# twosigma/Cook

Hardware: AMD Instinct MI355X
Metric: match-cycles/sec at 1M pending x 50k offers (higher is better)
Workload: dtype f64

## Files before the change

### cook_amd/csrc/classfit_asm.hpp

```cpp
#pragma once
#if CF_SLOTS_N == 12
#define CF_O_CTRL "13728"
#define CF_O_CTRL4 "13732"
#define CF_O_ARR "15280"
#define CF_O_CLS32 "9504"
#define CF_SLOT_SHIFT "9"
#define CF_SLOT_N "12"
#elif CF_SLOTS_N == 24
#define CF_O_CTRL "16800"
#define CF_O_CTRL4 "16804"
#define CF_O_ARR "18352"
#define CF_O_CLS32 "12576"
#define CF_SLOT_SHIFT "10"
#define CF_SLOT_N "24"
#else
#error "CF_SLOTS_N: 12 or 24"
#endif
#ifndef CF_ASM_WAIT_READS
#define CF_ASM_WAIT_READS "30"
#endif
#define CF_ASM_MAX_STEP(ctrl) "v_max_f32_dpp v113, v113, v113 " ctrl "\n\ts_nop 1\n\t"
#define CF_ASM_DECIDER_STEP                                                                                                             \
  "v_readlane_b32 s60, v80, s44\n\t"                                                                                                    \
  "v_readlane_b32 s61, v81, s44\n\t"                                                                                                    \
  "v_readlane_b32 s62, v82, s44\n\t"                                                                                                    \
  "s_mov_b32 s41, 1\n\t"                                                                                                                \
  "s_and_b32 s63, s62, 0xffff00ff\n\t"                                                                                                   \
  "s_cmp_lg_u32 s63, 0\n\t"                                                                                                             \
  "s_cbranch_scc1 9f\n\t"                                                                                                               \
                                                                                           \
  "v_mov_b32_e32 v88, s47\n\t"                                                                                                          \
  "v_mov_b32_e32 v89, s51\n\t"                                                                                                          \
  "v_add_u32_e32 v100, s46, v83\n\t"                                                                                                    \
  "s_mov_b64 exec, 1\n\t"                                                                                                               \
  "ds_write_b32 v89, v88 offset:" CF_O_CTRL4 "\n\t"                                                                                              \
  "s_mov_b64 exec, -1\n\t"                                                                                                              \
  "s_mov_b32 s82, " CF_ASM_WAIT_READS "\n\t"              \
  "1:\n\t"                                                                                                                              \
  "ds_read_b32 v92, v100\n\t"                                                                                                           \
  "ds_read_b64 v[94:95], v100 offset:8\n\t"                                                                                             \
  "ds_read_b128 v[96:99], v100 offset:16\n\t"                                                                                           \
  "ds_read_b32 v93, v100\n\t"                                                                                                           \
  "v_lshlrev_b32_e32 v114, 3, v65\n\t"  \
  "v_add_u32_e32 v114, s56, v114\n\t"                                                                                                   \
  "ds_read_b64 v[114:115], v114\n\t"                                                                                                    \
                                        \
  "v_subrev_u32_e32 v101, s60, v71\n\t"                                                                                                 \
  "v_subrev_u32_e32 v102, s61, v72\n\t"                                                                                                 \
  "v_cvt_f64_u32_e32 v[104:105], v101\n\t"                                                                                              \
  "v_cvt_f64_u32_e32 v[106:107], v102\n\t"                                                                                              \
  "v_mul_f64 v[104:105], v[104:105], v[66:67]\n\t"                                                                                      \
  "v_mul_f64 v[106:107], v[106:107], v[68:69]\n\t"                                                                                      \
  "v_add_f64 v[104:105], v[104:105], v[106:107]\n\t"                                                                                    \
  "v_add_f64 v[104:105], -v[104:105], 1.0\n\t"                                                                                          \
  "v_cmp_le_u32_e64 s[64:65], s60, v71\n\t"                                                                                             \
  "v_cmp_le_u32_e64 s[66:67], s61, v72\n\t"                                                                                             \
  "v_cmp_ne_u32_e64 s[68:69], 0, v64\n\t"                                                                                               \
  "s_and_b64 s[64:65], s[64:65], s[66:67]\n\t"                                                                                          \
  "s_and_b64 s[64:65], s[64:65], s[68:69]\n\t"                                                                                          \
  "s_waitcnt lgkmcnt(0)\n\t"                                                                                                            \
        \
  "s_bfe_u32 s63, s62, 0x4000c\n\t"                                                                                                     \
  "s_cmp_eq_u32 s63, 0\n\t"                                                                                                             \
  "s_cbranch_scc1 3f\n\t"                                                                                                               \
  "v_readlane_b32 s66, v85, s44\n\t"                                                                                                    \
  "v_readlane_b32 s67, v86, s44\n\t"                                                                                                    \
  "s_cmp_lt_u32 s63, 1\n\t"                                                                                                           \
  "s_cbranch_scc1 3f\n\t"                                                                                                               \
  "s_bfe_u32 s72, s66, 0x100000\n\t"                                                                      \
  "s_lshr_b32 s73, s72, 8\n\t"                                                                                                          \
  "s_lshl_b32 s73, s73, 3\n\t"                                                                                                          \
  "s_and_b32 s72, s72, 0xff\n\t"                                                                                                        \
  "v_lshrrev_b64 v[108:109], s73, v[114:115]\n\t"                                                                                       \
  "v_and_b32_e32 v108, 0xff, v108\n\t"                                                                                                  \
  "v_cmp_eq_u32_e64 s[74:75], s72, v108\n\t"                                                                                            \
  "s_and_b64 s[64:65], s[64:65], s[74:75]\n\t"                                                                                          \
  "s_cmp_lt_u32 s63, 2\n\t"                                                                                                           \
  "s_cbranch_scc1 3f\n\t"                                                                                                               \
  "s_bfe_u32 s72, s66, 0x100010\n\t"                                                                      \
  "s_lshr_b32 s73, s72, 8\n\t"                                                                                                          \
  "s_lshl_b32 s73, s73, 3\n\t"                                                                                                          \
  "s_and_b32 s72, s72, 0xff\n\t"                                                                                                        \
  "v_lshrrev_b64 v[108:109], s73, v[114:115]\n\t"                                                                                       \
  "v_and_b32_e32 v108, 0xff, v108\n\t"                                                                                                  \
  "v_cmp_eq_u32_e64 s[74:75], s72, v108\n\t"                                                                                            \
  "s_and_b64 s[64:65], s[64:65], s[74:75]\n\t"                                                                                          \
  "s_cmp_lt_u32 s63, 3\n\t"                                                                                                           \
  "s_cbranch_scc1 3f\n\t"                                                                                                               \
  "s_bfe_u32 s72, s67, 0x100000\n\t"                                                                      \
  "s_lshr_b32 s73, s72, 8\n\t"                                                                                                          \
  "s_lshl_b32 s73, s73, 3\n\t"                                                                                                          \
  "s_and_b32 s72, s72, 0xff\n\t"                                                                                                        \
  "v_lshrrev_b64 v[108:109], s73, v[114:115]\n\t"                                                                                       \
  "v_and_b32_e32 v108, 0xff, v108\n\t"                                                                                                  \
  "v_cmp_eq_u32_e64 s[74:75], s72, v108\n\t"                                                                                            \
  "s_and_b64 s[64:65], s[64:65], s[74:75]\n\t"                                                                                          \
  "s_cmp_lt_u32 s63, 4\n\t"                                                                                                           \
  "s_cbranch_scc1 3f\n\t"                                                                                                               \
  "s_bfe_u32 s72, s67, 0x100010\n\t"                                                                      \
  "s_lshr_b32 s73, s72, 8\n\t"                                                                                                          \
  "s_lshl_b32 s73, s73, 3\n\t"                                                                                                          \
  "s_and_b32 s72, s72, 0xff\n\t"                                                                                                        \
  "v_lshrrev_b64 v[108:109], s73, v[114:115]\n\t"                                                                                       \
  "v_and_b32_e32 v108, 0xff, v108\n\t"                                                                                                  \
  "v_cmp_eq_u32_e64 s[74:75], s72, v108\n\t"                                                                                            \
  "s_and_b64 s[64:65], s[64:65], s[74:75]\n\t"                                                                                          \
  "3:\n\t"                                                                                                                              \
   \
  "v_and_b32_e32 v108, 0xffffff00, v92\n\t"                                                                                             \
  "v_cmp_eq_u32_e64 s[70:71], s45, v108\n\t"                                                                                            \
  "v_cmp_eq_u32_e64 s[72:73], v92, v93\n\t"                                                                                             \
  "v_sub_u32_e32 v108, v73, v92\n\t"                                                                                                    \
  "v_and_b32_e32 v108, 0xff, v108\n\t"                                                                                                  \
  "v_cmp_gt_u32_e64 s[74:75], 3, v108\n\t"                                                                                              \
  "v_and_b32_e32 v109, 0xffff, v94\n\t"                                                                                                 \
  "v_cmp_ne_u32_e64 s[76:77], v109, v74\n\t"                                                                                            \
  "v_cmp_ne_u32_e64 s[78:79], v109, v75\n\t"                                                                                            \
  "v_cmp_gt_i32_e64 s[80:81], 0, v95\n\t"                                                                                               \
  "s_and_b64 s[74:75], s[74:75], s[76:77]\n\t"                                                                                          \
  "s_and_b64 s[74:75], s[74:75], s[78:79]\n\t"                                                                                          \
  "s_or_b64 s[74:75], s[74:75], s[80:81]\n\t"                                                                                           \
  "s_and_b64 s[72:73], s[70:71], s[72:73]\n\t"                                          \
  "s_and_b64 s[70:71], s[72:73], s[74:75]\n\t"                                                                                            \
  "s_andn2_b64 s[76:77], s[52:53], s[70:71]\n\t"                                                                     \
  "s_cmp_eq_u64 s[76:77], 0\n\t"                                                                                                          \
  "s_cbranch_scc1 2f\n\t"                                                                                                                 \
   \
   \
  "s_and_b64 s[78:79], s[76:77], s[72:73]\n\t"                                                                                            \
  "s_cmp_eq_u64 s[78:79], 0\n\t"                                                                                                          \
  "s_cbranch_scc1 4f\n\t"                                                                                                                 \
  "v_and_b32_e32 v109, 0x3fff, v95\n\t"                                                                                                   \
  "s_and_b64 s[72:73], s[64:65], s[54:55]\n\t"                                                   \
  "10:\n\t"                                                                                                                               \
  "s_ff1_i32_b64 s83, s[78:79]\n\t"                                                                                                       \
  "v_readlane_b32 s63, v109, s83\n\t"                                                                                                     \
  "s_bitset0_b64 s[78:79], s83\n\t"                                                                                                       \
  "v_cmp_eq_u32_e64 vcc, s63, v65\n\t"                                                                                                    \
  "s_and_b64 vcc, vcc, s[72:73]\n\t"                                                                                                      \
  "s_cmp_eq_u64 vcc, 0\n\t"                                                                                                               \
  "s_cbranch_scc1 11f\n\t"                                                                                                                \
  "s_bitset1_b64 s[80:81], s83\n\t"                                                                                                       \
  "s_bitset0_b64 s[76:77], s83\n\t"                                                                                                       \
  "11:\n\t"                                                                                                                               \
  "s_cmp_lg_u64 s[78:79], 0\n\t"                                                                                                          \
  "s_cbranch_scc1 10b\n\t"                                                                                                                \
  "s_cmp_eq_u64 s[76:77], 0\n\t"                                                                                                          \
  "s_cbranch_scc1 2f\n\t"                                                                                                                 \
  "4:\n\t"                                                                                                                                \
  "s_sub_u32 s82, s82, 1\n\t"      \
  "s_cmp_eq_u32 s82, 0\n\t"                                                                                                             \
  "s_cbranch_scc1 9f\n\t"                                                                                                               \
  "s_sleep 1\n\t"                                                                                                                       \
  "s_branch 1b\n\t"                                                                                                                     \
  "2:\n\t"                                                                                                                              \
  "s_andn2_b64 s[74:75], s[52:53], s[80:81]\n\t"                                                                        \
  "s_or_b64 s[64:65], s[64:65], s[74:75]\n\t"                                                          \
  "v_cndmask_b32_e64 v110, v98, v104, s[54:55]\n\t"                                                                                     \
  "v_cndmask_b32_e64 v111, v99, v105, s[54:55]\n\t"                                                                                     \
  "v_cndmask_b32_e64 v110, 0, v110, s[64:65]\n\t"                                                                                       \
  "v_cndmask_b32_e64 v111, 0, v111, s[64:65]\n\t"                                                                                       \
  "v_cvt_f32_f64_e32 v112, v[110:111]\n\t"                                                                                              \
  "s_nop 0\n\t"                                                                                                                         \
  "v_mov_b32_e32 v113, v112\n\t"                                                                                                        \
  "s_nop 1\n\t"                                                                                                                         \
  CF_ASM_MAX_STEP("quad_perm:[1,0,3,2] row_mask:0xf bank_mask:0xf")                                                                     \
  CF_ASM_MAX_STEP("quad_perm:[2,3,0,1] row_mask:0xf bank_mask:0xf")                                                                     \
  CF_ASM_MAX_STEP("row_half_mirror row_mask:0xf bank_mask:0xf")                                                                         \
  CF_ASM_MAX_STEP("row_mirror row_mask:0xf bank_mask:0xf")                                                                              \
  CF_ASM_MAX_STEP("row_bcast:15 row_mask:0xa bank_mask:0xf")                                                                            \
  CF_ASM_MAX_STEP("row_bcast:31 row_mask:0xc bank_mask:0xf")                                                                            \
  "v_readlane_b32 s63, v113, 63\n\t"                                                                                                    \
  "s_mov_b32 s41, 0\n\t"                                                                                                                \
  "s_cmp_eq_u32 s63, 0\n\t"                                                                                                             \
  "s_cbranch_scc1 9f\n\t"                                                                                          \
  "s_mov_b32 s41, 1\n\t"                                                                                                                \
  "v_cmp_eq_f32_e64 s[78:79], s63, v112\n\t"                                                                                            \
  "v_add_f32_e32 v108, 0x35000000, v112\n\t"                                                                               \
  "v_cmp_le_f32_e64 s[76:77], s63, v108\n\t"                                                                                            \
  "v_and_b32_e32 v109, 0x40000000, v95\n\t"                                                                                             \
  "v_cmp_ne_u32_e64 s[70:71], 0, v109\n\t"                                                                                              \
  "s_and_b64 s[76:77], s[76:77], s[64:65]\n\t"                                      \
  "s_bcnt1_i32_b64 s62, s[76:77]\n\t"                                                                                                   \
  "s_cmp_gt_u32 s62, 1\n\t"                                                                                                             \
  "s_cbranch_scc1 9f\n\t"                                                                                                               \
  "s_and_b64 s[70:71], s[70:71], s[76:77]\n\t"                                                                                          \
  "s_and_b64 s[70:71], s[70:71], s[74:75]\n\t"                       \
  "s_cmp_lg_u64 s[70:71], 0\n\t"                                                                                                        \
  "s_cbranch_scc1 9f\n\t"                                                                                                               \
  "s_ff1_i32_b64 s82, s[78:79]\n\t"                                                                                                     \
  "s_cmp_lt_u32 s82, 58\n\t"                                                                                                            \
  "s_cbranch_scc0 5f\n\t"                                                                                                               \
                                                                                                         \
  "v_readlane_b32 s64, v71, s82\n\t"                                                                                                    \
  "v_readlane_b32 s65, v72, s82\n\t"                                                                                                    \
  "v_readlane_b32 s66, v65, s82\n\t"                                                                                                    \
  "s_sub_u32 s67, s64, s60\n\t"                                                                                                         \
  "s_sub_u32 s70, s65, s61\n\t"                                                                                                         \
  "v_cmp_eq_u32_e64 vcc, s82, v84\n\t"                                                                                                  \
  "v_mov_b32_e32 v88, s67\n\t"                                                                                                          \
  "v_mov_b32_e32 v89, s70\n\t"                                                                                                          \
  "s_cmp_lt_u32 s67, s49\n\t"                                                                                                           \
  "s_cselect_b32 s71, 1, 0\n\t"                                                                                                         \
  "s_cmp_lt_u32 s70, s50\n\t"                                                                                                           \
  "s_cselect_b32 s62, 1, 0\n\t"                                                                                                         \
  "s_or_b32 s71, s71, s62\n\t"                                                                                                          \
  "v_cndmask_b32_e32 v71, v71, v88, vcc\n\t"                                                                                            \
  "v_cndmask_b32_e32 v72, v72, v89, vcc\n\t"                                                                                            \
  "s_cmp_lg_u32 s71, 0\n\t"                                                                                                             \
  "s_cselect_b64 s[62:63], vcc, 0\n\t"                             \
  "s_mov_b32 s72, s44\n\t"                                                                                                              \
  "s_mov_b32 s73, 0\n\t"                                                                                                                \
  "v_cndmask_b32_e64 v64, v64, 0, s[62:63]\n\t"                                                                                         \
  "s_branch 7f\n\t"                                                                                                                     \
        \
  "5:\n\t"                                                                                                                              \
  "v_readlane_b32 s64, v96, s82\n\t"                                                                                                    \
  "v_readlane_b32 s65, v97, s82\n\t"                                                                                                    \
  "v_readlane_b32 s76, v95, s82\n\t"                                                                                                    \
  "v_readlane_b32 s77, v94, s82\n\t"                                                                                                    \
  "v_readlane_b32 s78, v73, s82\n\t"                                                                                                    \
  "s_sub_u32 s67, s64, s60\n\t"                                                                                                         \
  "s_sub_u32 s70, s65, s61\n\t"                                                                                                         \
  "s_and_b32 s66, s76, 0x3fff\n\t"                                                                                                      \
  "s_bfe_u32 s79, s76, 0x80010\n\t"                                                                                                     \
  "s_and_b32 s73, s77, 0xffff\n\t"                                                                                                      \
  "s_lshr_b32 s81, s77, 16\n\t"                                                                                                         \
  "s_sub_u32 s80, s82, 57\n\t"                                                                                                          \
  "s_cmp_lt_u32 s67, s49\n\t"                                                                                                           \
  "s_cselect_b32 s71, 1, 0\n\t"                                                                                                         \
  "s_cmp_lt_u32 s70, s50\n\t"                                                                                                           \
  "s_cselect_b32 s62, 1, 0\n\t"                                                                                                         \
  "s_or_b32 s71, s71, s62\n\t"                                                                                                          \
  "s_bcnt1_i32_b64 s62, s[68:69]\n\t"                                                                                                   \
  "s_cmp_lg_u32 s71, 0\n\t"                                                                                                             \
  "s_cbranch_scc1 6f\n\t"                                                                                                               \
  "s_cmp_ge_u32 s62, " CF_ASM_EPOCH_LIVE "\n\t"                                                                                          \
  "s_cbranch_scc1 9f\n\t"                                  \
  "6:\n\t"                                                                                                                              \
  "s_lshl_b32 s62, s73, 3\n\t"                                                                                                          \
  "s_add_u32 s62, s62, s51\n\t"                                                                                                         \
  "s_lshl_b32 s63, s80, 2\n\t"                                                                                                          \
  "s_add_u32 s63, s63, s51\n\t"                                                                                                         \
  "s_add_u32 s78, s78, 1\n\t"                                                                                                           \
  "v_mov_b32_e32 v88, 0\n\t"                                                                                                            \
  "v_mov_b32_e32 v89, 0\n\t"                                                                                                            \
  "v_mov_b32_e32 v90, s62\n\t"                                                                                                          \
  "v_mov_b32_e32 v91, s63\n\t"                                                                                                          \
  "v_mov_b32_e32 v100, s78\n\t"                                                                                                         \
  "s_mov_b64 exec, 1\n\t"                                                                                                               \
  "ds_write_b64 v90, v[88:89] offset:" CF_O_ARR "\n\t"                                                                                         \
  "ds_write_b32 v91, v100 offset:" CF_O_CTRL4 "\n\t"                                                                                             \
  "s_mov_b64 exec, -1\n\t"                                                                                                              \
  "v_cmp_eq_u32_e64 vcc, s82, v84\n\t"                                                                                                  \
  "v_mov_b32_e32 v101, s73\n\t"                                                                                                         \
  "s_nop 0\n\t"                                                                                                                         \
  "v_cndmask_b32_e32 v75, v75, v74, vcc\n\t"                                                                                            \
  "v_cndmask_b32_e32 v74, v74, v101, vcc\n\t"                                                                                           \
  "v_cndmask_b32_e32 v73, v73, v100, vcc\n\t"                                                                                           \
  "s_lshl_b32 s62, s80, 8\n\t"                                                                                                          \
  "s_lshl_b32 s63, s81, 12\n\t"                                                                                                         \
  "s_or_b32 s72, s44, s62\n\t"                                                                                                          \
  "s_or_b32 s72, s72, s63\n\t"                                                                                                          \
  "s_cmp_lg_u32 s71, 0\n\t"                                                                                                             \
  "s_cbranch_scc1 7f\n\t"                                                                              \
  "s_mul_i32 s62, s79, 56\n\t"                                                                                                          \
  "s_add_u32 s62, s62, s51\n\t"                                                                                                         \
  "v_mov_b32_e32 v90, s62\n\t"                                                                                                          \
  "ds_read_b128 v[116:119], v90 offset:" CF_O_CLS32 "\n\t"                                                                                        \
  "s_andn2_b64 s[62:63], s[54:55], s[68:69]\n\t"                                                                                        \
  "s_ff1_i32_b64 s83, s[62:63]\n\t"                                                                                                     \
  "v_cmp_eq_u32_e64 vcc, s83, v84\n\t"                                                                                                  \
  "v_mov_b32_e32 v88, s66\n\t"                                                                                                          \
  "v_mov_b32_e32 v89, s79\n\t"                                                                                                          \
  "v_mov_b32_e32 v91, s67\n\t"                                                                                                          \
  "v_mov_b32_e32 v101, s70\n\t"                                                                                                         \
  "v_cndmask_b32_e64 v64, v64, 1, vcc\n\t"                                                                                              \
  "v_cndmask_b32_e32 v65, v65, v88, vcc\n\t"                                                                                            \
  "v_cndmask_b32_e32 v70, v70, v89, vcc\n\t"                                                                                            \
  "v_cndmask_b32_e32 v71, v71, v91, vcc\n\t"                                                                                            \
  "v_cndmask_b32_e32 v72, v72, v101, vcc\n\t"                                                                                           \
  "s_waitcnt lgkmcnt(0)\n\t"                                                                                                            \
  "v_cndmask_b32_e32 v66, v66, v116, vcc\n\t"                                                                                           \
  "v_cndmask_b32_e32 v67, v67, v117, vcc\n\t"                                                                                           \
  "v_cndmask_b32_e32 v68, v68, v118, vcc\n\t"                                                                                           \
  "v_cndmask_b32_e32 v69, v69, v119, vcc\n\t"                                                                                           \
   \
  "7:\n\t"                                                                                                                              \
  "v_cmp_eq_u32_e64 vcc, s44, v84\n\t"                                                                                                  \
  "v_mov_b32_e32 v88, s66\n\t"                                                                                                          \
  "v_cmp_lt_u32_e64 s[62:63], s67, v80\n\t"                                                                                             \
  "v_cmp_lt_u32_e64 s[76:77], s70, v81\n\t"                                                                                             \
  "v_cndmask_b32_e32 v76, v76, v88, vcc\n\t"                                                                                            \
  "s_or_b64 s[62:63], s[62:63], s[76:77]\n\t"                                                                                           \
  "s_lshl_b64 s[76:77], -2, s44\n\t"                                                                                                    \
  "s_and_b64 s[62:63], s[62:63], s[76:77]\n\t"                                                                                          \
  "s_or_b64 s[38:39], s[38:39], s[62:63]\n\t"                                                                                           \
  "s_min_u32 s37, s37, s67\n\t"                                                                                                         \
  "s_min_u32 s40, s40, s70\n\t"                                                                                                         \
  "s_add_u32 s36, s36, 1\n\t"                                                                                                           \
  "v_mov_b32_e32 v88, s72\n\t"                                                                                                          \
  "v_mov_b32_e32 v89, s73\n\t"                                                                                                          \
  "v_mov_b32_e32 v90, s64\n\t"                                                                                                          \
  "v_mov_b32_e32 v91, s65\n\t"                                                                                                          \
  "v_mov_b32_e32 v100, s48\n\t"                                                                                                         \
  "s_mov_b64 exec, 1\n\t"                                                                                                               \
  "ds_write_b128 v100, v[88:91]\n\t"                                                                                                    \
  "s_mov_b64 exec, -1\n\t"                                                                                                              \
  "s_mov_b32 s41, 2\n\t"                                                                                                                \
  "9:\n\t"

#define CF_ASM_CLASS_STEP                                                                                                               \
  "v_mov_b32_e32 v80, s44\n\t"                                                                                                          \
  "s_lshl_b32 s60, s45, 2\n\t"                                                                                                          \
  "s_add_u32 s60, s60, s44\n\t"                                                                                                         \
  "v_mov_b32_e32 v81, s60\n\t"                                                                                                          \
  "ds_read_b64 v[82:83], v80 offset:" CF_O_CTRL "\n\t"                                                                     \
  "ds_read_b32 v84, v81 offset:" CF_O_CTRL4 "\n\t"                                                                   \
  "s_mov_b32 s41, 3\n\t"                                                                                                                \
  "s_waitcnt lgkmcnt(0)\n\t"                                                                                                            \
  "v_readfirstlane_b32 s61, v82\n\t"                                                                                                    \
  "v_readfirstlane_b32 s42, v83\n\t"                                                                                                    \
  "v_readfirstlane_b32 s43, v84\n\t"                                                                                                    \
  "s_cmp_lg_u32 s61, 0\n\t"                                                                                                             \
  "s_cbranch_scc1 9f\n\t"                                                                                                               \
  "s_cmp_lg_u32 s43, s40\n\t"                                                                                                           \
  "s_cbranch_scc1 9f\n\t"                                                                                                               \
  "s_mov_b32 s41, 2\n\t"                                                                                                                \
                                                                                                 \
  "1:\n\t"                                                                                                                              \
  "s_cmp_eq_u64 s[36:37], 0\n\t"                                                                                                        \
  "s_cbranch_scc1 9f\n\t"                                                                                                               \
  "s_cmp_eq_u32 s39, s56\n\t"                                                                                                           \
  "s_cbranch_scc1 2f\n\t"                                                                                                               \
  "s_add_u32 s62, s36, -1\n\t"                                                                                                          \
  "s_addc_u32 s63, s37, -1\n\t"                                                                                                         \
  "s_and_b64 s[36:37], s[36:37], s[62:63]\n\t"                                                                                          \
  "s_add_u32 s38, s38, 1\n\t"                                                                                                           \
  "s_add_u32 s39, s39, 1\n\t"                                                                                                           \
  "s_cmp_eq_u32 s39, s57\n\t"                                                                                                           \
  "s_cselect_b32 s39, 0, s39\n\t"                                                                                                       \
  "s_branch 1b\n\t"                                                                                                                     \
  "2:\n\t"                                                                                                                                \
  "s_lshr_b32 s60, s42, 8\n\t"                                                                                                            \
  "s_cmp_lt_u32 s38, s60\n\t"                                          \
  "s_cbranch_scc0 12f\n\t"                                                                                                                \
  "s_mov_b32 s41, 3\n\t"                                                                                                                  \
  "s_branch 9f\n\t"                                                                                                                       \
  "12:\n\t"                                                                                                                               \
  "s_add_u32 s60, s60, s59\n\t"                                                                                                         \
  "s_cmp_ge_u32 s38, s60\n\t"                                                                                                           \
  "s_cbranch_scc1 9f\n\t"                                                                             \
  "s_ff1_i32_b64 s64, s[36:37]\n\t"                                                                                                     \
  "v_readlane_b32 s65, v72, s64\n\t"                                                                                                    \
  "v_readlane_b32 s66, v73, s64\n\t"                                                                                                    \
  "v_readlane_b32 s67, v74, s64\n\t"                                                                                                    \
  "s_mov_b32 s41, 1\n\t"                                                                                                                \
  "s_lshr_b32 s60, s67, 12\n\t"                                                                                                         \
  "s_cmp_lg_u32 s60, 0\n\t"                                                                                                             \
  "s_cbranch_scc1 9f\n\t"                                                                                \
  "s_and_b32 s60, s67, 0xff\n\t"                                                                                                        \
  "s_cmp_lg_u32 s60, s58\n\t"                                                                                                           \
  "s_cbranch_scc1 8f\n\t"                                                                                \
                                           \
  "s_bfe_u32 s60, s67, 0x30008\n\t"                                                                                                     \
  "s_bitcmp1_b32 s60, 0\n\t"                                                                                                            \
  "s_cselect_b64 vcc, -1, 0\n\t"                                                                                                        \
  "v_cndmask_b32_e32 v80, v64, v65, vcc\n\t"                                                                                            \
  "v_cndmask_b32_e32 v81, v66, v67, vcc\n\t"                                                                                            \
  "v_cndmask_b32_e32 v82, v68, v69, vcc\n\t"                                                                                            \
  "v_cndmask_b32_e32 v83, v70, v71, vcc\n\t"                                                                                            \
  "s_bitcmp1_b32 s60, 1\n\t"                                                                                                            \
  "s_cselect_b64 vcc, -1, 0\n\t"                                                                                                        \
  "v_cndmask_b32_e32 v80, v80, v81, vcc\n\t"                                                                                            \
  "v_cndmask_b32_e32 v82, v82, v83, vcc\n\t"                                                                                            \
  "s_bitcmp1_b32 s60, 2\n\t"                                                                                                            \
  "s_cselect_b64 vcc, -1, 0\n\t"                                                                                                        \
  "v_cndmask_b32_e32 v80, v80, v82, vcc\n\t"                                                                                            \
                                                                 \
  "s_mul_i32 s68, s38, 43\n\t"                                                                                                          \
  "s_lshr_b32 s68, s68, " CF_SLOT_SHIFT "\n\t"                                                                                                          \
  "s_mul_i32 s68, s68, " CF_SLOT_N "\n\t"                                                                                                          \
  "s_sub_u32 s68, s38, s68\n\t"                                                                                                         \
  "s_lshl_b32 s68, s68, 8\n\t"                                                                                                          \
  "s_lshl_b32 s69, s45, 5\n\t"                                                                                                          \
  "s_add_u32 s68, s68, s69\n\t"                                                                                                         \
  "s_add_u32 s68, s68, s44\n\t"                                                                                                         \
  "s_add_u32 s69, s46, s64\n\t"                                                                                                         \
  "s_lshl_b32 s69, s69, 12\n\t"                                                                                                         \
  "s_or_b32 s69, s69, s47\n\t"                                                                                                          \
  "s_and_b32 s70, s40, 0xff\n\t"                                                                                                        \
  "s_or_b32 s69, s69, s70\n\t"                                                                                                          \
  "v_mov_b32_e32 v94, s68\n\t"                                                                                                          \
  "v_mov_b32_e32 v95, s69\n\t"                                                                                                          \
  "v_mov_b32_e32 v96, -1\n\t"                                                                                                           \
  "v_cmp_lt_u32_e64 s[70:71], s66, v80\n\t"                                                 \
  "s_cmp_eq_u64 s[70:71], 0\n\t"                                                                                                        \
  "s_cbranch_scc1 6f\n\t"                                                                                                               \
  "s_ff1_i32_b64 s72, s[70:71]\n\t"                                                                                                     \
  "s_lshl_b32 s73, s72, 6\n\t"                                                                                                          \
  "s_add_u32 s74, s73, s48\n\t"                                                                        \
  "s_sub_u32 s75, s49, s73\n\t"                                                                              \
  "v_add_u32_e32 v97, s74, v75\n\t"                                                                                                     \
  "v_lshlrev_b32_e32 v98, 3, v97\n\t"                                                                                                   \
  "v_add_u32_e32 v98, s44, v98\n\t"                                                                                                     \
  "v_lshlrev_b32_e32 v99, 1, v97\n\t"                                                                                                   \
  "v_add_u32_e32 v99, s50, v99\n\t"                                                                                                     \
  "ds_read_b64 v[84:85], v98 offset:" CF_O_ARR "\n\t"                                                                                          \
  "ds_read_u16 v90, v99\n\t"                                                                                                            \
  "s_waitcnt lgkmcnt(0)\n\t"                                                                                                            \
  "v_cmp_le_u32_e64 s[76:77], s65, v84\n\t"                                                                                             \
  "v_cmp_le_u32_e64 s[78:79], s66, v85\n\t"                                                                                             \
  "v_cmp_gt_u32_e64 s[80:81], s75, v75\n\t"                                                                                             \
  "v_and_b32_e32 v91, 0x8000, v90\n\t"                                                                                                  \
  "v_cmp_eq_u32_e64 s[82:83], 0, v91\n\t"                                                                                               \
  "s_and_b64 s[76:77], s[76:77], s[78:79]\n\t"                                                                                          \
  "s_and_b64 s[76:77], s[76:77], s[80:81]\n\t"                                                                                          \
  "s_and_b64 s[76:77], s[76:77], s[82:83]\n\t"                                                                                          \
  "s_cmp_eq_u64 s[76:77], 0\n\t"                                                                                                        \
  "s_cbranch_scc1 9f\n\t"               \
                                                    \
  "v_subrev_u32_e32 v91, s65, v84\n\t"                                                                                                  \
  "v_subrev_u32_e32 v92, s66, v85\n\t"                                                                                                  \
  "v_cvt_f64_u32_e32 v[86:87], v91\n\t"                                                                                                 \
  "v_cvt_f64_u32_e32 v[88:89], v92\n\t"                                                                                                 \
  "v_mul_f64 v[86:87], v[86:87], s[52:53]\n\t"                                                                                          \
  "v_mul_f64 v[88:89], v[88:89], s[54:55]\n\t"                                                                                          \
  "v_add_f64 v[86:87], v[86:87], v[88:89]\n\t"                                                                                          \
  "v_add_f64 v[86:87], -v[86:87], 1.0\n\t"                                                                                              \
  "v_mov_b32_e32 v91, s72\n\t"                                                                                                          \
  "v_lshl_or_b32 v92, v91, 16, v97\n\t"                                                                \
  "v_and_b32_e32 v93, 0x3fff, v90\n\t"                                                                                                  \
  "v_or_b32_e32 v93, s51, v93\n\t"                                                                                                      \
  "v_lshlrev_b32_e32 v91, 16, v90\n\t"                                                                                                  \
  "v_and_b32_e32 v91, 0x40000000, v91\n\t"                              \
  "v_or_b32_e32 v93, v93, v91\n\t"                                                                                                      \
  "s_ff1_i32_b64 s78, s[76:77]\n\t"                                                                                                     \
  "s_lshl_b64 s[78:79], 1, s78\n\t"                                                                                                     \
  "s_mov_b64 exec, s[78:79]\n\t"                                                                                                        \
  "ds_write_b32 v94, v96\n\t"                                                                                                           \
  "ds_write_b128 v94, v[84:87] offset:16\n\t"                                                                                           \
  "ds_write_b64 v94, v[92:93] offset:8\n\t"                                                                                             \
  "ds_write_b32 v94, v95\n\t"                                                                                                           \
  "s_mov_b64 exec, -1\n\t"                                                                                                              \
  "s_branch 8f\n\t"                                                                                                                     \
                                                                                                    \
  "6:\n\t"                                                                                                                              \
  "v_mov_b32_e32 v92, 0\n\t"                                                                                                            \
  "v_mov_b32_e32 v93, 0x80000000\n\t"                                                                                                   \
  "s_mov_b64 exec, 1\n\t"                                                                                                               \
  "ds_write_b32 v94, v96\n\t"                                                                                                           \
  "ds_write_b64 v94, v[92:93] offset:8\n\t"                                                                                             \
  "ds_write_b32 v94, v95\n\t"                                                                                                           \
  "s_mov_b64 exec, -1\n\t"                                                                                                              \
                                                                                                              \
  "8:\n\t"                                                                                                                              \
  "s_add_u32 s62, s36, -1\n\t"                                                                                                          \
  "s_addc_u32 s63, s37, -1\n\t"                                                                                                         \
  "s_and_b64 s[36:37], s[36:37], s[62:63]\n\t"                                                                                          \
  "s_add_u32 s38, s38, 1\n\t"                                                                                                           \
  "s_add_u32 s39, s39, 1\n\t"                                                                                                           \
  "s_cmp_eq_u32 s39, s57\n\t"                                                                                                           \
  "s_cselect_b32 s39, 0, s39\n\t"                                                                                                       \
  "s_mov_b32 s41, 0\n\t"                                                                                                                \
  "9:\n\t"
```

### cook_amd/csrc/classfit_host.hpp

```cpp

static int classfit_env() {
  static const int v = [] {
    const char* s = std::getenv("COOK_CLASSFIT");
    return s && (s[0] == '0' || s[0] == '1') ? s[0] - '0' : -1;
  }();
  return v;
}
static bool classfit_by_default(const cook_engine* e) {
  const int f = classfit_env();
  if (f >= 0) return f == 1;
  return g_engines_on_device[e->device & 63].load() >= 6;
}
static size_t cf_lds_bytes_host(unsigned NP, unsigned M, bool eq, unsigned G, unsigned S) {
  size_t n = sizeof(CfFixed) + (size_t)NP * 10u;
  n = (n + 7u) & ~(size_t)7u;
  if (eq) n += (size_t)M * 8u;
  n += ((size_t)G + 1u) * 2u + (size_t)G * 2u + (size_t)S * 2u;
  return n + 64u;
}
bool cf_setup(cook_engine* e, const MatchIn& in, const MatchIn* in_dev, const MatchState& st, const JobRec* jr, const JobCons* jcons, const OfferA* oa, const OfferB* ob,
              CfPoolCtx& ctx) {
  const unsigned K = in.K, M = in.M, G = in.G;
  e->cf_inelig = 0x10000u;
  if (K == 0 || M == 0 || M > CF_SORT_N || G > CF_MAXG || in.good_enough < 1.0 || in.has_x || in.reserved_bits || in.host_dup) return false;
  if (e->cf_max_host == 0xFFFFFFFFu || (size_t)e->cf_max_host > 8u * (size_t)M + 65536u) return false;
  CfBuf b{};
  b.ctl = e->cf_ctl.ensure(1);
  b.jr = jr, b.jcons = jcons, b.oa = oa, b.ob = ob;
  b.attr8 = e->cf_attr8.ensure(M);
  b.max_host = e->cf_max_host;
  b.h2o = e->cf_h2o.ensure((size_t)b.max_host + 1u);
  b.pos_fc = e->cf_pos[0].ensure(M), b.pos_fm = e->cf_pos[1].ensure(M), b.pos_cid = e->cf_pos[2].ensure(M);
  b.scr_fc = e->cf_scr[0].ensure(M), b.scr_fm = e->cf_scr[1].ensure(M), b.scr_cid = e->cf_scr[2].ensure(M);
  b.jobs = e->cf_jobs.ensure(K);
  b.gcount = e->cf_gcount.ensure(std::max(1u, G));
  b.gmem = e->cf_gmem.ensure((size_t)std::max(1u, G) * CF_GMEM);
  static_assert(sizeof(CfCtl) % 4 == 0, "cf_init clears the control block word by word");
  KM<cf_init, 256>(e, "cf_init", std::min(div_up(b.max_host + 1u, 1024u), 512u), b, b.max_host + 1u, std::max(1u, G));
  KM<cf_scan, 256>(e, "cf_scan", div_up(std::max(K, M), 256), in_dev, b, K, M);
  KM<cf_prepare, 1024>(e, "cf_prepare", 1u, in_dev, b, st.jmin, K, M, G, in.host_dup, in.reserved_bits ? 1u : 0u);
  KM<cf_pack_jobs, 256>(e, "cf_pack_jobs", div_up(K, 256), in_dev, b, K);
  static_assert(offsetof(CfCtl, t) <= 512, "the control block's head is read back through the 512-byte scratch");
  pinned_copy(e, e->h_scratch, b.ctl, offsetof(CfCtl, t), hipMemcpyDeviceToHost);
  sync(e);
  CfCtl hc;
  std::memcpy((void*)&hc, e->h_scratch, offsetof(CfCtl, t));
  e->cf_inelig = hc.inelig;
  if (hc.inelig) return false;
  const unsigned NP = (M + 63u) & ~63u;
  const unsigned S = hc.any_group ? e->cf_group_run_total + hc.n_grouped : 0u;
  if (cf_lds_bytes_host(NP, M, hc.any_eq != 0u, hc.any_group ? G : 0u, S) > CF_LDS_BYTES || S > 60000u) {
    e->cf_inelig = CF_X_SHAPE;
    return false;
  }
  ctx.in = in_dev;
  ctx.st = st;
  ctx.b = b;
  return true;
}
static void cf_prof_print(const uint32_t* q) {
#ifdef CF_PROF
  std::fprintf(stderr, "CFPROF (x16 shader cycles) decider: slow steps %u (candidates %u evaluation %u commit %u) plain steps %u in %u walk-total %u | class wave 1: poll %u answer %u answers %u idle %u idles %u | class wave 2: poll %u answer %u answers %u idle %u idles %u | walk ticks(100MHz) %u | batch boundaries: decider %u, batches without a walked job %u\n", q[27], q[24], q[25], q[26], q[28], q[29], q[31], q[32], q[33], q[35], q[36], q[37], q[40], q[41], q[43], q[44], q[45], q[CFS_TICKS_WALK], q[30], q[38]);
#else
  (void)q;
#endif
}
void cf_run(cook_engine* lead, cook_engine* const* es, unsigned n, hipStream_t stream) {
  cook_engine* e = lead;
  for (unsigned i0 = 0; i0 < n; i0 += (unsigned)CF_PACK) {
    const unsigned c = std::min<unsigned>(CF_PACK, n - i0);
    CfPack pk{};
    for (unsigned x = 0; x < (unsigned)CF_PACK; ++x) pk.c[x] = es[i0 + (x < c ? x : 0u)]->placement.walk;
    KLS("cf_walk", stream, cf_walk, c, CF_THREADS, pk);
  }
  for (unsigned i = 0; i < n; ++i) {
    const CfPoolCtx& c = es[i]->placement.walk;
    const unsigned G = es[i]->last_in.G;
    if (G) KLS("cf_group_chains", stream, cf_group_chains, div_up(G, 256), 256, c.b, c.st, G);
  }
  constexpr size_t SLOT = 16 + 48 * 4;
  if (!lead->h_cf) COOK_HIP(hipHostMalloc((void**)&lead->h_cf, 64 * SLOT, hipHostMallocDefault));
  for (unsigned i = 0; i < n; ++i) {
    char* slot = lead->h_cf + i * SLOT;
    COOK_HIP(hipMemcpyAsync(slot, es[i]->placement.walk.st.summary, 16, hipMemcpyDeviceToHost, stream));
    COOK_HIP(hipMemcpyAsync(slot + 16, es[i]->placement.walk.b.ctl->stats, 48 * 4, hipMemcpyDeviceToHost, stream));
  }
  COOK_HIP(hipStreamSynchronize(stream));
  for (unsigned i = 0; i < n; ++i) {
    cook_engine* x = es[i];
    const unsigned* sum = (const unsigned*)(lead->h_cf + i * SLOT);
    if (sum[3] == 0xDEADu) lead->fail(COOK_E_STATE, "cf_walk: the pool's tables do not fit the workgroup's LDS (the host's check let it through)");
    std::memcpy(x->cf_stats, lead->h_cf + i * SLOT + 16, 48 * 4);
    cf_prof_print(x->cf_stats);
    WinCtl c{};
    c.matched = sum[0], c.head_matched = sum[1], c.rounds = sum[2], c.head = x->last_in.K, c.visited_sum = x->cf_stats[CFS_WALKED];
    c.t_seq = x->cf_stats[CFS_TICKS_TOTAL], c.t_setup = x->cf_stats[CFS_TICKS_PROLOGUE];
    x->placement_complete(3, c);
  }
}
```

### cook_amd/csrc/classfit_walk.hpp

```cpp
#pragma once
#if defined(CF_PROF) && !defined(CF_STATS)
#define CF_STATS 1
#endif
#ifdef CF_STATS
#define CF_STAT(x) x
#define CF_TICKS() cook_ticks()
#else
#define CF_STAT(x) ((void)0)
#define CF_TICKS() 0ull
#endif
#ifdef CF_PROF
#define CF_PROF_T(x) const unsigned long long x = __builtin_readcyclecounter()
#define CF_PROF_ADD(i, d) prof[i] += (unsigned long long)(d)
#else
#define CF_PROF_T(x) ((void)0)
#define CF_PROF_ADD(i, d) ((void)0)
#endif

#ifndef CF_AHEAD
#define CF_AHEAD 10
#endif
constexpr unsigned CF_BOARD = CF_AHEAD;
#ifndef CF_SLOTS_N
#define CF_SLOTS_N 12
#endif
constexpr unsigned CF_SLOTS = CF_SLOTS_N;
static_assert(CF_BOARD + 2u <= CF_SLOTS, "a slot is free again before its wave writes it two rows on");
static_assert(CF_SLOTS == 12u || CF_SLOTS == 24u, "cf_slot and classfit_asm.hpp know these two");
static __device__ __forceinline__ unsigned cf_slot(unsigned ord) { return ord - CF_SLOTS * ((ord * 43u) >> (CF_SLOTS == 12u ? 9 : 10)); }
constexpr unsigned CF_OVL = 58;
constexpr unsigned CF_EPOCH_AT = COOK_SHAPE(58, 8);
constexpr unsigned CFW_BOOKS = 4;
enum : unsigned { CFM_EXACT = 1u, CFM_EPOCH = 2u, CFM_BATCH_END = 3u };
enum : unsigned { CFX_NEXT_BASE = 0, CFX_SPARE1, CFX_LOGN, CFX_LOG_APPLIED, CFX_WALK_LO, CFX_WALK_HI, CFX_EX_LANE, CFX_FMAX_LO, CFX_FMAX_HI, CFX_EPOCH, CFX_MATCH_LO, CFX_MATCH_HI,
                  CFX_B1_LO, CFX_B1_HI, CFX_OVN, CFX_MINFC, CFX_MINFM, CFX_N = 24 };
constexpr uint32_t CF_ENT_NONE = 0x80000000u, CF_ENT_AMB = 0x40000000u;

struct __attribute__((aligned(8))) CfFree {
  uint32_t c, m;
};
struct CfEnt {
  uint32_t tag, pad, pos, cid;
  uint32_t fc, fm;
  double fa;
};
struct CfLog {
  uint32_t info, pos;
  uint32_t ofc, ofm, nfc, nfm, pad0, pad1;
};
struct CfPost {
  double fa;
  uint32_t w0;
  uint32_t pos;
  uint32_t fc, fm, cls, aux;
};
struct CfJobU {
  unsigned c, m, kind, L, n_eq, n_nov, grouped, grp, eq0, eq1, nov0, nov1;
};
struct CfLds {
  CfFree* fcm;
  uint16_t* cid;
  CfEnt* board;
  CfLog* log;
  uint32_t* ctrl;
  uint64_t* attr8;
  uint16_t *goff, *gcnt, *gids;
  CfJob* ring;
  CfPost* post2;
  CfClass* cls;
  uint32_t* pw;
  uint32_t* aw;
  uint32_t* gk;
  uint32_t* ovt;
  uint32_t* ovl;
  uint32_t* ckept;
  uint32_t* misc;
  const uint32_t* t;
  const uint32_t* envw;
};

struct CfLv8 {
  uint32_t v0, v1, v2, v3, v4, v5, v6, v7;
};
#define CF_FOR8(F) F(0) F(1) F(2) F(3) F(4) F(5) F(6) F(7)
static __device__ __forceinline__ unsigned cf_level_of(const uint32_t* t, uint32_t fc) {
  unsigned n = 0;
#pragma unroll
  for (int i = 0; i < CF_LV; ++i) n += fc >= t[i] ? 1u : 0u;
  return n;
}
static_assert(CF_LV == 8, "CfLv8 holds the call's levels");
static __device__ __forceinline__ CfLv8 cf_levels_load(const uint32_t* t) {
  const uint32_t t0 = t[0], t1 = t[1], t2 = t[2], t3 = t[3], t4 = t[4], t5 = t[5], t6 = t[6], t7 = t[7];
  return CfLv8{wave_uniform_u32(t0), wave_uniform_u32(t1), wave_uniform_u32(t2), wave_uniform_u32(t3), wave_uniform_u32(t4), wave_uniform_u32(t5), wave_uniform_u32(t6), wave_uniform_u32(t7)};
}
static __device__ __forceinline__ unsigned cf_level_of(const CfLv8& t, uint32_t fc) {
  unsigned n = 0;
#define CF_LO(i) n += fc >= t.v##i ? 1u : 0u;
  CF_FOR8(CF_LO)
#undef CF_LO
  return n;
}
static __device__ __forceinline__ uint32_t cf_lv_get(const CfLv8& a, unsigned i) {
  const bool b0 = (i & 1u) != 0u, b1 = (i & 2u) != 0u, b2 = (i & 4u) != 0u;
  const uint32_t r01 = b0 ? a.v1 : a.v0, r23 = b0 ? a.v3 : a.v2, r45 = b0 ? a.v5 : a.v4, r67 = b0 ? a.v7 : a.v6;
  const uint32_t r03 = b1 ? r23 : r01, r47 = b1 ? r67 : r45;
  return b2 ? r47 : r03;
}
struct CfChunkLane {
  unsigned cls, kind, pos0, n, Tc, Tm;
  unsigned long long dE;
  double hTc, hTm;
  CfLv8 lv, la;
};

static __device__ __forceinline__ void cf_setup_chunks(const CfClass* cls, unsigned nc, unsigned lw, unsigned lane, CfChunkLane& c, unsigned& nch_wave) {
  c.cls = 0xFFu, c.kind = 0xFEu, c.pos0 = 0u, c.n = 0u, c.Tc = 1u, c.Tm = 1u, c.dE = 0ull, c.hTc = 0.0, c.hTm = 0.0;
  unsigned acc = 0;
  for (unsigned ci = 0; ci < nc; ++ci) {
    const CfClass& cl = cls[ci];
    if (cl.wave != lw) continue;
    const unsigned nch = (cl.n + 63u) / 64u;
    if (lane >= acc && lane < acc + nch) {
      const unsigned x = lane - acc;
      c.cls = ci, c.kind = cl.kind, c.pos0 = cl.off + 64u * x, c.n = cf_min(64u, cl.n - 64u * x), c.Tc = cl.Tc, c.Tm = cl.Tm, c.dE = cl.dE, c.hTc = cl.hTc, c.hTm = cl.hTm;
    }
    acc += nch;
  }
  nch_wave = acc;
}

static __device__ __forceinline__ void cf_tighten(const CfLds& S, const CfLv8& t, unsigned lane, unsigned ch, CfChunkLane& c) {
  const unsigned pos0 = (unsigned)wave_read_lane((int)c.pos0, (int)ch), n = (unsigned)wave_read_lane((int)c.n, (int)ch);
  const bool in = lane < n;
  const CfFree f = S.fcm[pos0 + lane];
  const uint32_t cid = S.cid[pos0 + lane];
  const unsigned nl = in ? cf_level_of(t, f.c) : 0u;
  const bool free_host = !(cid & CF_OCC);
#define CF_TI_A(i) unsigned a##i = nl > (unsigned)i ? f.m + 1u : 0u;
#define CF_TI_R(i) unsigned r##i = (nl > (unsigned)i && free_host) ? f.m + 1u : 0u;
  CF_FOR8(CF_TI_A)
  CF_FOR8(CF_TI_R)
#undef CF_TI_A
#undef CF_TI_R
  wave_max8_u32(a0, a1, a2, a3, a4, a5, a6, a7);
  wave_max8_u32(r0, r1, r2, r3, r4, r5, r6, r7);
#define CF_TI_S(i) \
  if (lane == ch) c.la.v##i = a##i, c.lv.v##i = r##i;
  CF_FOR8(CF_TI_S)
#undef CF_TI_S
}
static __device__ __forceinline__ void cf_wave_tables(const CfLds& S, unsigned lw, unsigned lane, const CfChunkLane& c, unsigned kinds, unsigned n_kind) {
#define CF_TB_P(i) unsigned p##i = c.kind == 0u ? c.lv.v##i : 0u;
#define CF_TB_A(i) unsigned a##i = c.kind < 0xFEu ? c.la.v##i : 0u;
  CF_FOR8(CF_TB_P)
  CF_FOR8(CF_TB_A)
#undef CF_TB_P
#undef CF_TB_A
  wave_max8_u32(p0, p1, p2, p3, p4, p5, p6, p7);
  wave_max8_u32(a0, a1, a2, a3, a4, a5, a6, a7);
  st_lane0_b128(&S.pw[lw * CF_LV], p0, p1, p2, p3), st_lane0_b128(&S.pw[lw * CF_LV + 4], p4, p5, p6, p7);
  st_lane0_b128(&S.aw[lw * CF_LV], a0, a1, a2, a3), st_lane0_b128(&S.aw[lw * CF_LV + 4], a4, a5, a6, a7);
  for (unsigned k = 1; k < n_kind; ++k) {
    if (!((kinds >> k) & 1u)) continue;
#define CF_TB_G(i) unsigned g##i = c.kind == k ? c.lv.v##i : 0u;
    CF_FOR8(CF_TB_G)
#undef CF_TB_G
    wave_max8_u32(g0, g1, g2, g3, g4, g5, g6, g7);
    st_lane0_b128(&S.gk[k * CF_LV], g0, g1, g2, g3), st_lane0_b128(&S.gk[k * CF_LV + 4], g4, g5, g6, g7);
  }
  WAIT_LDS();
}

static __device__ __forceinline__ bool cf_cons_ok(const CfLds& S, const CfJobU& J, unsigned id, bool active) {
  bool ok = true;
  if (J.n_eq) {
    const uint64_t a8 = S.attr8[active ? id : 0u];
#pragma unroll
    for (unsigned q = 0; q < 4u; ++q) {
      const unsigned e = ((q < 2u ? J.eq0 : J.eq1) >> (16u * (q & 1u))) & 0xFFFFu;
      if (q < J.n_eq) ok = ok && (unsigned)((a8 >> (8u * (e >> 8))) & 255ull) == (e & 255u);
    }
  }
  if (J.n_nov) {
#pragma unroll
    for (unsigned q = 0; q < 4u; ++q) {
      const unsigned h = ((q < 2u ? J.nov0 : J.nov1) >> (16u * (q & 1u))) & 0xFFFFu;
      if (q < J.n_nov) ok = ok && id != h;
    }
  }
  if (J.grouped) {
    const unsigned g0 = S.goff[J.grp], gn = ld_wg(&S.gcnt[J.grp]);
    for (unsigned x = 0; x < gn; ++x) ok = ok && id != (unsigned)S.gids[g0 + x];
  }
  return ok;
}
static __device__ __forceinline__ double cf_literal(unsigned Tc, unsigned Tm, unsigned fc, unsigned fm, unsigned jc, unsigned jm, double sc, double sm) {
  const double A = (double)(Tc - fc) * sc, Bm = (double)(Tm - fm) * sm, c = (double)jc * sc, m = (double)jm * sm;
  return ((A + c) / ((double)Tc * sc) + (Bm + m) / ((double)Tm * sm)) / 2.0;
}

struct CfAns {
  bool have, amb;
  unsigned pos, ch, cid, fc, fm, cls;
  double fa;
};
static __device__ __forceinline__ void cf_class_answer(const CfLds& S, const CfLv8& tl, const CfJobU& J, unsigned lane, CfChunkLane& c, CfAns& out, unsigned& scans,
                                                       unsigned& tightened) {
  out.have = false, out.amb = false, out.pos = 0u, out.ch = 0u, out.cid = 0u, out.fc = 0u, out.fm = 0u, out.cls = 0u, out.fa = 0.0;
  const uint32_t lvL = cf_lv_get(c.lv, J.L);
  unsigned long long m = __ballot(c.kind == J.kind && lvL > J.m);
  while (m) {
    const unsigned ch = (unsigned)__ffsll(m) - 1u;
    ++scans;
    const unsigned pos0 = (unsigned)wave_read_lane((int)c.pos0, (int)ch), n = (unsigned)wave_read_lane((int)c.n, (int)ch);
    const unsigned q = pos0 + lane;
    const CfFree f = S.fcm[q];
    const uint32_t cid = S.cid[q];
    const bool room = lane < n && f.c >= J.c && f.m >= J.m && !(cid & CF_OCC);
    const bool ok = room && cf_cons_ok(S, J, cid & CF_IDMASK, room);
    const unsigned long long b = __ballot(ok);
    if (b == 0ull) {
      if (__ballot(room) == 0ull) {
        cf_tighten(S, tl, lane, ch, c);
        ++tightened;
      }
      m &= ~(1ull << ch);
      continue;
    }
    const unsigned q0 = (unsigned)__ffsll(b) - 1u;
    const unsigned fc0 = (unsigned)wave_read_lane((int)f.c, (int)q0), fm0 = (unsigned)wave_read_lane((int)f.m, (int)q0), cid0 = (unsigned)wave_read_lane((int)cid, (int)q0);
    const unsigned cls = (unsigned)wave_read_lane((int)c.cls, (int)ch);
    m &= ~__ballot(c.cls == cls);
    const bool tie = (cid0 & CF_TIE) != 0u;
    const double hTc = wave_read_lane_f64(c.hTc, (int)ch), hTm = wave_read_lane_f64(c.hTm, (int)ch);
    const double f0 = 1.0 - ((double)(fc0 - J.c) * hTc + (double)(fm0 - J.m) * hTm);
    if (!out.have || f0 > out.fa + CF_BAND) out.amb = tie;
    else if (f0 >= out.fa - CF_BAND) out.amb = true;
    if (!out.have || f0 > out.fa) out.fa = f0, out.cid = cid0 & CF_IDMASK, out.pos = pos0 + q0, out.fc = fc0, out.fm = fm0, out.cls = cls, out.ch = ch;
    out.have = true;
  }
}
static __device__ __forceinline__ void cf_class_query_exact(const CfLds& S, const CfJobU& J, unsigned lane, const CfChunkLane& c, double fmax, double sc, double sm, CfPost& out,
                                                            unsigned& scans) {
  out.fa = 0.0, out.w0 = 0u, out.pos = 0u, out.fc = 0u, out.fm = 0u, out.cls = 0u, out.aux = 0u;
  const uint32_t lvL = cf_lv_get(c.lv, J.L);
  unsigned long long m = __ballot(c.kind == J.kind && lvL > J.m);
  unsigned long long best_lit = 0ull;
  while (m) {
    const unsigned ch = (unsigned)__ffsll(m) - 1u;
    ++scans;
    const unsigned pos0 = (unsigned)wave_read_lane((int)c.pos0, (int)ch), n = (unsigned)wave_read_lane((int)c.n, (int)ch);
    const unsigned Tc = (unsigned)wave_read_lane((int)c.Tc, (int)ch), Tm = (unsigned)wave_read_lane((int)c.Tm, (int)ch), cls = (unsigned)wave_read_lane((int)c.cls, (int)ch);
    const double hTc = wave_read_lane_f64(c.hTc, (int)ch), hTm = wave_read_lane_f64(c.hTm, (int)ch);
    const unsigned q = pos0 + lane;
    const CfFree f = S.fcm[q];
    const uint32_t cid = S.cid[q];
    const bool room = lane < n && f.c >= J.c && f.m >= J.m && !(cid & CF_OCC);
    const bool ok = room && cf_cons_ok(S, J, cid & CF_IDMASK, room);
    const double fa = ok ? 1.0 - ((double)(f.c - J.c) * hTc + (double)(f.m - J.m) * hTm) : 0.0;
    const bool cand = ok && fa >= fmax - CF_BAND;
    const double lit = cand ? cf_literal(Tc, Tm, f.c, f.m, J.c, J.m, sc, sm) : 0.0;
    const unsigned long long lb = (unsigned long long)__double_as_longlong(lit);
    const unsigned long long mx = wave_max_u64(lb);
    if (mx != 0ull) {
      const unsigned idmin = ~wave_max_u32((cand && lb == mx) ? ~(cid & CF_IDMASK) : 0u);
      if (mx > best_lit || (mx == best_lit && idmin < out.w0)) {
        best_lit = mx;
        const unsigned q0 = (unsigned)__ffsll(__ballot(cand && lb == mx && (cid & CF_IDMASK) == idmin)) - 1u;
        out.fa = __longlong_as_double((long long)mx), out.w0 = idmin, out.pos = pos0 + q0, out.fc = (unsigned)wave_read_lane((int)f.c, (int)q0),
        out.fm = (unsigned)wave_read_lane((int)f.m, (int)q0), out.cls = cls, out.aux = ch;
      }
    }
    m &= ~(1ull << ch);
  }
}

struct CfOvLane {
  unsigned valid, id, cls, fc, fm;
  double hTc, hTm;
};
static __device__ __forceinline__ void cf_overlay_query_exact(const CfLds& S, const CfJobU& J, unsigned lane, const CfOvLane& o, double fmax, double sc, double sm, CfPost& out) {
  out.fa = 0.0, out.w0 = 0u, out.pos = 0u, out.fc = 0u, out.fm = 0u, out.cls = 0u, out.aux = 0u;
  if (J.kind != 0u) return;
  const bool isov = lane < CF_OVL;
  const bool room = isov && o.valid && o.fc >= J.c && o.fm >= J.m;
  const bool ok = room && cf_cons_ok(S, J, o.id, room);
  const double fa = ok ? 1.0 - ((double)(o.fc - J.c) * o.hTc + (double)(o.fm - J.m) * o.hTm) : 0.0;
  const bool cand = ok && fa >= fmax - CF_BAND;
  const unsigned Tc = S.cls[isov && o.valid ? o.cls : 0u].Tc, Tm = S.cls[isov && o.valid ? o.cls : 0u].Tm;
  const double lit = cand ? cf_literal(Tc, Tm, o.fc, o.fm, J.c, J.m, sc, sm) : 0.0;
  const unsigned long long lb = (unsigned long long)__double_as_longlong(lit);
  const unsigned long long mx = wave_max_u64(lb);
  if (mx == 0ull) return;
  const unsigned idmin = ~wave_max_u32((cand && lb == mx) ? ~o.id : 0u);
  const unsigned l0 = (unsigned)__ffsll(__ballot(cand && lb == mx && o.id == idmin)) - 1u;
  out.fa = __longlong_as_double((long long)mx), out.w0 = idmin, out.pos = l0, out.fc = (unsigned)wave_read_lane((int)o.fc, (int)l0),
  out.fm = (unsigned)wave_read_lane((int)o.fm, (int)l0), out.cls = (unsigned)wave_read_lane((int)o.cls, (int)l0);
}
struct CfVerdict {
  int src;
  unsigned id, pos, fc, fm, cls, aux;
};
static __device__ __forceinline__ CfVerdict cf_verdict_exact(const CfPost* posts, unsigned lane, unsigned used_sets) {
  CfVerdict v;
  const bool has = lane == 0u || (lane < 7u && ((used_sets >> lane) & 1u));
  CfPost p;
  p.fa = 0.0, p.w0 = 0u, p.pos = p.fc = p.fm = p.cls = p.aux = 0u;
  if (has) p = posts[lane];
  const unsigned long long fb = (unsigned long long)__double_as_longlong(p.fa);
  const unsigned long long mx = wave_max_u64(fb);
  v.src = -1, v.id = v.pos = v.fc = v.fm = v.cls = v.aux = 0u;
  if (mx == 0ull) return v;
  const unsigned idmin = ~wave_max_u32((has && fb == mx) ? ~p.w0 : 0u);
  const unsigned wl = (unsigned)__ffsll(__ballot(has && fb == mx && p.w0 == idmin)) - 1u;
  v.src = (int)wl;
  v.id = (unsigned)wave_read_lane((int)p.w0, (int)wl), v.pos = (unsigned)wave_read_lane((int)p.pos, (int)wl), v.fc = (unsigned)wave_read_lane((int)p.fc, (int)wl),
  v.fm = (unsigned)wave_read_lane((int)p.fm, (int)wl), v.cls = (unsigned)wave_read_lane((int)p.cls, (int)wl), v.aux = (unsigned)wave_read_lane((int)p.aux, (int)wl);
  return v;
}
static __device__ __forceinline__ unsigned cf_poll(const uint32_t* p) { return (unsigned)wave_read_lane((int)ld_wg(p), 0); }
static __device__ __forceinline__ unsigned long long cf_below(unsigned s) { return (1ull << s) - 1ull; }

enum : unsigned { CFE_K = 0, CFE_M, CFE_NP, CFE_NCLS, CFE_NKIND, CFE_CMIN, CFE_MMIN, CFE_KC, CFE_KM, CFE_MINFC, CFE_MINFM, CFE_N = 12 };
constexpr float CF_BAND32 = 1.0f / 2097152.0f;

struct CfFixed {
  CfEnt board[CF_SLOTS * 8u];
  CfLog log[64];
  CfJob ring[2u * 64u];
  CfPost post2[8];
  CfClass cls[CF_MAXCLS];
  uint32_t pw[8u * CF_LV], aw[8u * CF_LV], gk[CF_MAXKIND * CF_LV], ovt[CF_LV];
  uint32_t ctrl[8];
  uint32_t ovl[192], ckept[3u * CF_MAXCLS], misc[CFX_N];
  uint32_t env_t[CF_LV], envw[CFE_N];
};
static_assert(sizeof(CfFixed) % 16 == 0, "the arrays behind it are 16-byte aligned");
static_assert(offsetof(CfFixed, pw) % 16 == 0 && offsetof(CfFixed, aw) % 16 == 0 && offsetof(CfFixed, gk) % 16 == 0 && (CF_LV * 4) % 16 == 0, "cf_wave_tables stores the rows 16 bytes at a time");
#if COOK_HAS_ASM_WALK
#define CF_ASM_EPOCH_LIVE "57"
#include "classfit_asm.hpp"
static_assert(CF_EPOCH_AT == 58 && CF_OVL == 58, "classfit_asm.hpp: the overlay's size");
static_assert(offsetof(CfFixed, ctrl) == 13728 + (CF_SLOTS - 12) * 256 && offsetof(CfFixed, cls) == 9472 + (CF_SLOTS - 12) * 256 && sizeof(CfFixed) == 15280 + (CF_SLOTS - 12) * 256 && sizeof(CfClass) == 56 && offsetof(CfClass, hTc) == 32 &&
                  offsetof(CfClass, hTm) == 40 && offsetof(CfEnt, pos) == 8 && offsetof(CfEnt, cid) == 12 && offsetof(CfEnt, fc) == 16 && offsetof(CfEnt, fa) == 24 && sizeof(CfEnt) == 32 &&
                  sizeof(CfLog) == 32 && offsetof(CfLog, ofc) == 8,
              "classfit_asm.hpp: offsets of the LDS records");
typedef unsigned cf_u32x16 __attribute__((ext_vector_type(16)));
typedef unsigned cf_u32x8 __attribute__((ext_vector_type(8)));
typedef unsigned cf_u32x4 __attribute__((ext_vector_type(4)));
#endif

template <int ROLE>
static __device__ __forceinline__ void cf_walk_role(const CfLds& S, const MatchState& st, const CfBuf& b, const unsigned lw, const unsigned rep, const unsigned nrep,
                                                    const unsigned long long t_start) {
  constexpr bool is_decider = ROLE == 0, is_class_wave = ROLE == 1, is_books = ROLE == 2;
  const unsigned tid = threadIdx.x, lane = lane_id();
  CfCtl* ctl = b.ctl;
  const unsigned K = wave_uniform_u32(S.envw[CFE_K]), cmin = wave_uniform_u32(S.envw[CFE_CMIN]), mmin = wave_uniform_u32(S.envw[CFE_MMIN]);
  const uint32_t* t = S.t;
  CfLv8 tl = CfLv8{0u, 0u, 0u, 0u, 0u, 0u, 0u, 0u};
  if (is_class_wave) tl = cf_levels_load(t);
#define n_cls wave_uniform_u32(S.envw[CFE_NCLS])
#define n_kind wave_uniform_u32(S.envw[CFE_NKIND])
#define NP wave_uniform_u32(S.envw[CFE_NP])
  CfChunkLane c;
  unsigned nch_wave = 0;
  cf_setup_chunks(S.cls, n_cls, is_class_wave ? lw : 0xFFu, lane, c, nch_wave);
  c.lv = CfLv8{0u, 0u, 0u, 0u, 0u, 0u, 0u, 0u}, c.la = c.lv;
  unsigned my_kinds = 0;
  {
    const unsigned forw = is_class_wave ? lw : (is_decider && lane >= CF_OVL ? lane - CF_OVL + 1u : 0xFFu);
    for (unsigned ci = 0; ci < n_cls; ++ci)
      if (S.cls[ci].wave == forw && S.cls[ci].kind < 32u) my_kinds |= 1u << S.cls[ci].kind;
  }
  const unsigned wk = is_class_wave ? wave_uniform_u32(my_kinds) : 0u;
  unsigned one_cls = 0xFFFFFFFFu, u_off = 0, u_n = 0;
  double u_hTc = 0.0, u_hTm = 0.0;
  auto class_setup = [&] {
    unsigned cnt = 0, ci0 = 0;
    for (unsigned ci = 0; ci < n_cls; ++ci)
      if (S.cls[ci].wave == lw) ++cnt, ci0 = ci;
    one_cls = cnt == 1u ? ci0 : 0xFFFFFFFFu;
    const CfClass* cl = &S.cls[ci0];
    u_off = cl->off, u_n = cl->n, u_hTc = cl->hTc, u_hTm = cl->hTm;
  };
  if (is_class_wave) {
    class_setup();
    for (unsigned ch = 0; ch < nch_wave; ++ch) cf_tighten(S, tl, lane, ch, c);
    if (rep == 0u && lw != 0u) cf_wave_tables(S, lw, lane, c, wk, n_kind);
  }
  CfOvLane o;
  o.valid = 0u, o.id = 0u, o.cls = 0u, o.fc = 0u, o.fm = 0u, o.hTc = 0.0, o.hTm = 0.0;
  unsigned nrm = 0, rm1 = 0xFFFFFFFFu, rm2 = 0xFFFFFFFFu;
  unsigned minfc_all = wave_uniform_u32(S.envw[CFE_MINFC]), minfm_all = wave_uniform_u32(S.envw[CFE_MINFM]);
  unsigned matched = 0, head = 0;
  unsigned jc = 0, jm = 0, jmeta = 0, jgrp = 0, jeq0 = 0, jeq1 = 0, jnov0 = 0, jnov1 = 0;
  int res = -1;
  unsigned long long b1m = 0ull;
  unsigned seen = 0, gen = 0;
  unsigned tight_applied = 0;
  bool bk_room0 = false, nx_room0 = false, nx_walk = false;
  unsigned st_scans = 0, st_exact = 0, st_open = 0, st_ovwin = 0, st_gpu = 0, st_epochs = 0, st_tight = 0, st_walked = 0, st_dead = 0, st_opendead = 0, st_spins = 0, st_flips = 0,
           st_rewinds = 0;
  unsigned long long tk_epoch = 0, tk_books = 0, tk_walk = 0, tk_phase1 = 0;
#ifdef CF_PROF
  unsigned long long prof[8] = {0, 0, 0, 0, 0, 0, 0, 0}, bnd0 = 0ull;
#endif
  auto job_of = [&](unsigned s) -> CfJobU {
    CfJobU J;
    J.c = (unsigned)wave_read_lane((int)jc, (int)s), J.m = (unsigned)wave_read_lane((int)jm, (int)s);
    const unsigned meta = (unsigned)wave_read_lane((int)jmeta, (int)s);
    J.kind = meta & 255u, J.L = (meta >> 8) & 15u, J.n_eq = (meta >> 12) & 15u, J.n_nov = (meta >> 16) & 15u, J.grouped = (meta >> 20) & 1u;
    J.grp = 0u, J.eq0 = J.eq1 = 0u, J.nov0 = J.nov1 = 0xFFFFFFFFu;
    if (meta >> 12) {
      J.grp = (unsigned)wave_read_lane((int)jgrp, (int)s), J.eq0 = (unsigned)wave_read_lane((int)jeq0, (int)s), J.eq1 = (unsigned)wave_read_lane((int)jeq1, (int)s),
      J.nov0 = (unsigned)wave_read_lane((int)jnov0, (int)s), J.nov1 = (unsigned)wave_read_lane((int)jnov1, (int)s);
    }
    return J;
  };
  auto tables_room_any = [&](unsigned L, unsigned m) -> bool {
    bool r = S.ovt[L] > m;
    for (unsigned x = 1; x <= (unsigned)CF_CW; ++x) r = r || S.aw[x * CF_LV + L] > m;
    return r;
  };
  auto tables_walk = [&](unsigned kind, unsigned L, unsigned m) -> bool {
    bool r = false;
    if (kind == 0u) {
      r = S.ovt[L] > m;
      for (unsigned x = 1; x <= (unsigned)CF_CW; ++x) r = r || S.pw[x * CF_LV + L] > m;
    } else if (kind < (unsigned)CF_MAXKIND) {
      r = S.gk[kind * CF_LV + L] > m;
    }
    return r;
  };
  CfJob nxt;
  nxt.c = nxt.m = nxt.meta = nxt.grp = nxt.eq[0] = nxt.eq[1] = nxt.nov[0] = nxt.nov[1] = 0u;
  constexpr unsigned CF_PRE = 3;
  CfJob pre[CF_PRE];
  auto books_next = [&](unsigned nbase) -> unsigned long long {
    const unsigned nn = nbase < K ? cf_min(64u, K - nbase) : 0u;
    const unsigned nslot = (nbase >> 6) & 1u;
    const bool in = lane < nn;
    if (in) S.ring[nslot * 64u + lane] = nxt;
    const unsigned kind = nxt.meta & 255u, L = (nxt.meta >> 8) & 15u;
    nx_room0 = in && tables_room_any(L, nxt.m);
    nx_walk = in && tables_walk(kind, L, nxt.m);
    const unsigned long long wm = __ballot(nx_walk);
    if (lane == 0)
      S.misc[CFX_WALK_LO] = (unsigned)wm, S.misc[CFX_WALK_HI] = (unsigned)(wm >> 32), S.misc[CFX_LOGN] = 0u, S.misc[CFX_LOG_APPLIED] = 0u,
      S.ctrl[1] = wm ? (unsigned)__ffsll(wm) - 1u : 0u;
    return wm;
  };
  auto books_advance = [&](unsigned nbase) {
    nxt = pre[0];
#pragma unroll
    for (unsigned i = 0; i + 1u < CF_PRE; ++i) pre[i] = pre[i + 1u];
    if (nbase + 64u * (CF_PRE + 1u) + lane < K) pre[CF_PRE - 1u] = b.jobs[nbase + 64u * (CF_PRE + 1u) + lane];
  };
  __syncthreads();
  if (is_books) {
    if (lane < cf_min(64u, K)) nxt = b.jobs[lane];
    books_next(0u);
    bk_room0 = nx_room0;
    if (64u + lane < K) nxt = b.jobs[64u + lane];
#pragma unroll
    for (unsigned i = 0; i < CF_PRE; ++i) {
      pre[i] = nxt;
      if (64u * (i + 2u) + lane < K) pre[i] = b.jobs[64u * (i + 2u) + lane];
    }
  }
  if (is_decider) cook_set_prio_high();
  const unsigned long long t_loop = cook_ticks();
  __syncthreads();
  const bool isov = lane < CF_OVL;
  const unsigned clw = isov ? 0u : lane - CF_OVL + 1u;

  for (unsigned base = 0; base < K;) {
    const unsigned bn = cf_min(64u, K - base);
    const unsigned slot = (base >> 6) & 1u;
    const unsigned long long walkmask = wave_uniform_u64((unsigned long long)S.misc[CFX_WALK_LO] | (unsigned long long)S.misc[CFX_WALK_HI] << 32);
    const unsigned nw = (unsigned)__popcll(walkmask);
    st_walked += nw;
    if (!is_books) {
      const CfJob j = S.ring[slot * 64u + (lane < bn ? lane : 0u)];
      const bool in = lane < bn;
      jc = in ? j.c : 0u, jm = in ? j.m : 0u, jmeta = in ? j.meta : CF_KIND_NONE, jgrp = j.grp, jeq0 = j.eq[0], jeq1 = j.eq[1], jnov0 = j.nov[0], jnov1 = j.nov[1];
    }
    res = -1;
    if (is_decider) b1m = __ballot(!(jc <= minfc_all && jm <= minfm_all));
    unsigned logn = 0;
    unsigned long long todo = walkmask;
    unsigned cur_ord = 0;
    unsigned ph = 0;
    bool batch_done = nw == 0u;
    auto decider_books = [&](unsigned n_placed) {
      if (lane < bn) st.job_to_offer[base + lane] = res;
      const unsigned long long mm = __ballot(res >= 0);
      if (base == 0u) head = (unsigned)(mm & 1ull);
      const bool live = isov && o.valid != 0u;
      const unsigned nl = live ? cf_level_of(t, o.fc) : 0u;
#define CF_OV_T(i) unsigned v##i = nl > (unsigned)i ? o.fm + 1u : 0u;
      CF_FOR8(CF_OV_T)
#undef CF_OV_T
      wave_max8_u32(v0, v1, v2, v3, v4, v5, v6, v7);
      if (lane == 0) {
        S.misc[CFX_MATCH_LO] = (unsigned)mm, S.misc[CFX_MATCH_HI] = (unsigned)(mm >> 32), S.misc[CFX_B1_LO] = (unsigned)b1m, S.misc[CFX_B1_HI] = (unsigned)(b1m >> 32);
        S.misc[CFX_LOGN] = n_placed, S.misc[CFX_MINFC] = minfc_all, S.misc[CFX_MINFM] = minfm_all;
#define CF_OV_S(i) S.ovt[i] = v##i;
        CF_FOR8(CF_OV_S)
#undef CF_OV_S
      }
    };
    const unsigned long long tw0 = CF_TICKS();
    CF_PROF_T(cw0);
#ifdef CF_PROF
    if (is_decider && nw != 0u && bnd0 != 0ull) prof[6] += cw0 - bnd0, bnd0 = 0ull;
    if (is_class_wave && nw == 0u) prof[6] += 16ull;
#endif
    while (!batch_done) {
      unsigned md = 0;
      if (is_decider) {
#if COOK_HAS_ASM_WALK
        cf_u32x16 ST = {0u, 0u, 0u, 0u, 0u, 0u, 0u, 0u, 0u, 0u, 0u, 0u, 0u, 0u, 0u, 0u};
        cf_u32x8 JB = {jc, jm, jmeta, clw * 32u, lane, jeq0, jeq1, 0u};
        const unsigned long long rel0 = cook_ballot(!isov & ((my_kinds & 1u) != 0u)), ovm = cf_below(CF_OVL);
        const cf_u32x8 MK = {wave_uniform_u32((unsigned)rel0), wave_uniform_u32((unsigned)(rel0 >> 32)), wave_uniform_u32((unsigned)ovm), wave_uniform_u32((unsigned)(ovm >> 32)),
                             wave_uniform_u32(cook_lds_off(S.attr8)), 0u, 0u, 0u};
        const unsigned a_board = wave_uniform_u32(cook_lds_off(S.board)), a_log = wave_uniform_u32(cook_lds_off(S.log));
        auto st_pack = [&] {
          const unsigned long long hc = (unsigned long long)__double_as_longlong(o.hTc), hm = (unsigned long long)__double_as_longlong(o.hTm);
          ST[0] = o.valid, ST[1] = o.id, ST[2] = (unsigned)hc, ST[3] = (unsigned)(hc >> 32), ST[4] = (unsigned)hm, ST[5] = (unsigned)(hm >> 32), ST[6] = o.cls, ST[7] = o.fc, ST[8] = o.fm,
          ST[9] = nrm, ST[10] = rm1, ST[11] = rm2, ST[12] = (unsigned)res;
        };
        auto st_unpack = [&] {
          o.valid = ST[0], o.id = ST[1], o.hTc = __longlong_as_double((long long)((unsigned long long)ST[3] << 32 | ST[2])),
          o.hTm = __longlong_as_double((long long)((unsigned long long)ST[5] << 32 | ST[4])), o.cls = ST[6], o.fc = ST[7], o.fm = ST[8], nrm = ST[9], rm1 = ST[10], rm2 = ST[11],
          res = (int)ST[12];
        };
#endif
        while (md == 0u) {
          todo = wave_uniform_u64(todo), cur_ord = wave_uniform_u32(cur_ord), logn = wave_uniform_u32(logn), matched = wave_uniform_u32(matched), gen = wave_uniform_u32(gen);
          minfc_all = wave_uniform_u32(minfc_all), minfm_all = wave_uniform_u32(minfm_all), b1m = wave_uniform_u64(b1m);
#if COOK_HAS_ASM_WALK
          {
            st_pack();
            CF_PROF_T(f0);
            while (todo != 0ull) {
              const unsigned fs = (unsigned)__ffsll(todo) - 1u;
#define CF_U(x) wave_uniform_u32((unsigned)(x))
              cf_u32x8 SC = {CF_U(matched), CF_U(minfc_all), CF_U(b1m), CF_U(b1m >> 32), CF_U(minfm_all), 1u, 0u, 0u};
              const cf_u32x8 AR = {CF_U(fs), CF_U((base + fs) << 12 | (gen & 15u) << 8), CF_U(a_board + cf_slot(cur_ord) * 8u * (unsigned)sizeof(CfEnt)), CF_U(fs | cur_ord << 8),
                                   CF_U(a_log + logn * (unsigned)sizeof(CfLog)), CF_U(cmin), CF_U(mmin), a_board};
#undef CF_U
              asm volatile(CF_ASM_DECIDER_STEP
                           : "+{v[64:79]}"(ST), "+{s[36:43]}"(SC)
                           : "{v[80:87]}"(JB), "{s[44:51]}"(AR), "{s[52:59]}"(MK)
                           : "v88", "v89", "v90", "v91", "v92", "v93", "v94", "v95", "v96", "v97", "v98", "v99", "v100", "v101", "v102", "v103", "v104", "v105", "v106", "v107", "v108",
                             "v109", "v110", "v111", "v112", "v113", "v114", "v115", "v116", "v117", "v118", "v119", "s60", "s61", "s62", "s63", "s64", "s65", "s66", "s67", "s68", "s69",
                             "s70", "s71", "s72", "s73", "s74", "s75", "s76", "s77", "s78", "s79", "s80", "s81", "s82", "s83", "vcc", "scc", "memory");
#ifdef CF_DELAY_D
              __builtin_amdgcn_s_sleep(6);
#endif
              const unsigned status = wave_uniform_u32(SC[5]);
              if (status == 1u) break;
              matched = wave_uniform_u32(SC[0]), minfc_all = wave_uniform_u32(SC[1]), minfm_all = wave_uniform_u32(SC[4]);
              b1m = wave_uniform_u64((unsigned long long)SC[3] << 32 | SC[2]);
              logn += status >> 1;
              todo &= todo - 1ull, ++cur_ord;
              CF_PROF_ADD(4, 1);
            }
            CF_PROF_T(f1);
            CF_PROF_ADD(5, f1 - f0);
            WAIT_LDS();
            st_unpack();
          }
#endif
          if (todo == 0ull) {
#ifdef CF_PROF
            bnd0 = __builtin_readcyclecounter();
#endif
            decider_books(logn);
            md = CFM_BATCH_END;
            st_lane0_b32(&S.ctrl[0], md);
            break;
          }
          CF_PROF_T(p0);
          const unsigned s = (unsigned)__ffsll(todo) - 1u;
          const unsigned ord = cur_ord;
          st_lane0_b32(&S.ctrl[1], s | ord << 8);
          const unsigned Jc = (unsigned)wave_read_lane((int)jc, (int)s), Jm = (unsigned)wave_read_lane((int)jm, (int)s), meta = (unsigned)wave_read_lane((int)jmeta, (int)s);
          const unsigned kind = meta & 255u;
          const unsigned want = (base + s) << 12 | (gen & 15u) << 8;
          const CfEnt* e = &S.board[cf_slot(ord) * 8u + clw];
          const bool relevant = !isov && kind < 32u && ((my_kinds >> (kind & 31u)) & 1u);
          unsigned cpos, ccid, cfc, cfm;
          double cfa;
          bool acc;
          bool ok_ov = isov & (o.valid != 0u) & (kind == 0u) & (o.fc >= Jc) & (o.fm >= Jm);
          if (meta >> 12) {
            const CfJobU J = job_of(s);
            ok_ov = ok_ov & cf_cons_ok(S, J, o.id, ok_ov);
          }
          for (;;) {
            const unsigned t1 = ld_wg(&e->tag);
            COMPILER_FENCE();
            cpos = e->pos, ccid = e->cid, cfc = e->fc, cfm = e->fm, cfa = e->fa;
            COMPILER_FENCE();
            const unsigned t2 = ld_wg(&e->tag);
            const unsigned behind = (nrm - t1) & 255u, p = cpos & 0xFFFFu;
            const bool ours = (t1 == t2) & ((t1 & ~255u) == want);
            acc = ours & (((ccid & CF_ENT_NONE) != 0u) | ((behind <= 2u) & (p != rm1) & (p != rm2)));
            if (cook_ballot(relevant & !acc) == 0ull) break;
            for (unsigned long long rq = cook_ballot(relevant & !acc & ours); rq != 0ull; rq &= rq - 1ull) {
              const unsigned L = (unsigned)__ffsll(rq) - 1u;
              const unsigned xid = (unsigned)wave_read_lane((int)(ccid & CF_IDMASK), (int)L);
              if (cook_ballot(ok_ov & (o.id == xid)) != 0ull && lane == L) acc = true, ccid = CF_ENT_NONE;
            }
            if (cook_ballot(relevant & !acc) == 0ull) break;
            CF_STAT(++st_spins);
            SPIN_PAUSE_NEAR();
          }
          CF_PROF_T(p1);
          CF_PROF_ADD(0, p1 - p0);
          const unsigned vfc = isov ? o.fc : cfc, vfm = isov ? o.fm : cfm, vid = isov ? o.id : (ccid & CF_IDMASK);
          const bool vvalid = isov ? (o.valid != 0u && kind == 0u) : (relevant && !(ccid & CF_ENT_NONE));
          const bool room = vvalid & (vfc >= Jc) & (vfm >= Jm);
          const bool ok = isov ? ok_ov : room;
          double fov = 1.0 - ((double)(vfc - Jc) * o.hTc + (double)(vfm - Jm) * o.hTm);
          OPAQUE_V(fov);
          const double fa = ok ? (isov ? fov : cfa) : 0.0;
          const float ff = (float)fa;
          const float mx = wave_max_f32(ff);
          const unsigned long long eqm = cook_ballot(ok & (ff == mx)), nearm = cook_ballot(ok & (ff >= mx - CF_BAND32)),
                                   ambm = cook_ballot(ok & !isov & ((ccid & CF_ENT_AMB) != 0u) & (ff >= mx - CF_BAND32));
          CF_PROF_T(p2);
          CF_PROF_ADD(1, p2 - p1);
          CF_PROF_ADD(3, 1);
          if (!(mx > 0.0f)) {
            todo &= todo - 1ull, ++cur_ord;
            continue;
          }
          unsigned l0 = (unsigned)__ffsll(eqm) - 1u;
          if ((nearm & (nearm - 1ull)) != 0ull || ambm != 0ull) {
            const unsigned long long mxb = wave_max_u64((unsigned long long)__double_as_longlong(fa));
            const double f0 = __longlong_as_double((long long)mxb);
            l0 = (unsigned)__ffsll(__ballot(ok && (unsigned long long)__double_as_longlong(fa) == mxb)) - 1u;
            const unsigned long long near = __ballot(ok && fa >= f0 - CF_BAND);
            const bool amb = (near & (near - 1ull)) != 0ull || (__ballot(ok && !isov && (ccid & CF_ENT_AMB) && fa >= f0 - CF_BAND) != 0ull);
            if (amb) {
              md = CFM_EXACT;
              if (lane == 0) S.misc[CFX_EX_LANE] = s, S.misc[CFX_FMAX_LO] = (unsigned)mxb, S.misc[CFX_FMAX_HI] = (unsigned)(mxb >> 32), st_wg(&S.ctrl[0], md);
              break;
            }
          }
          todo &= todo - 1ull, ++cur_ord;
          const unsigned ofc = (unsigned)wave_read_lane((int)vfc, (int)l0), ofm = (unsigned)wave_read_lane((int)vfm, (int)l0), id = (unsigned)wave_read_lane((int)vid, (int)l0);
          const unsigned nfc = ofc - Jc, nfm = ofm - Jm;
          const bool dead = nfc < cmin || nfm < mmin;
          const bool from_ov = l0 < CF_OVL;
          ++matched;
          res = lane == s ? (int)id : res;
          b1m |= cook_ballot((jc > nfc) | (jm > nfm)) & ~cf_below(s) & ~(1ull << s);
          minfc_all = cf_min(minfc_all, nfc), minfm_all = cf_min(minfm_all, nfm);
          unsigned lpos = 0, linfo = s;
          if (from_ov) {
            CF_STAT(++st_ovwin);
            const bool me = lane == l0;
            o.fc = me ? nfc : o.fc, o.fm = me ? nfm : o.fm, o.valid = (me && dead) ? 0u : o.valid;
            if (dead) CF_STAT(++st_dead);
          } else {
            const bool gpu_place = kind != 0u;
            const unsigned pos = (unsigned)wave_read_lane((int)cpos, (int)l0);
            const unsigned cls2 = ((unsigned)wave_read_lane((int)ccid, (int)l0) >> 16) & 255u;
            const unsigned cw = l0 - CF_OVL + 1u;
            const unsigned cnt2 = (unsigned)wave_read_lane((int)nrm, (int)l0) + 1u;
            lpos = pos & 0xFFFFu, linfo = s | cw << 8 | (pos >> 16) << 12 | (gpu_place ? 1u : 0u) << 20;
            if (gpu_place) {
              st_lane0_b64(&S.fcm[lpos], nfc, nfm);
              if (lane == 0) S.cid[lpos] = (uint16_t)(S.cid[lpos] | CF_OCC);
              CF_STAT(++st_gpu);
            } else {
              st_lane0_b64(&S.fcm[lpos], 0u, 0u);
            }
            st_lane0_b32(&S.ctrl[1u + cw], cnt2);
            const bool me = lane == l0;
            rm2 = me ? rm1 : rm2, rm1 = me ? lpos : rm1, nrm = me ? cnt2 : nrm;
            if (!gpu_place && !dead) {
              CF_STAT(++st_open);
              const unsigned long long vm = cook_ballot(isov & (o.valid != 0u));
              const unsigned lf = (unsigned)__ffsll(~(vm | ~cf_below(CF_OVL))) - 1u;
              const CfClass* cl = &S.cls[cls2];
              const double hTc2 = cl->hTc, hTm2 = cl->hTm;
              const bool nl = lane == lf;
              o.valid = nl ? 1u : o.valid, o.id = nl ? id : o.id, o.cls = nl ? cls2 : o.cls, o.fc = nl ? nfc : o.fc, o.fm = nl ? nfm : o.fm, o.hTc = nl ? hTc2 : o.hTc,
              o.hTm = nl ? hTm2 : o.hTm;
              const unsigned live1 = wave_uniform_u32((unsigned)__popcll(vm) + 1u);
              if (live1 >= CF_EPOCH_AT) md = CFM_EPOCH;
            } else if (!gpu_place) {
              CF_STAT(++st_opendead);
            }
          }
          st_lane0_b128(&S.log[logn].info, linfo, lpos, ofc, ofm);
          ++logn;
          if ((meta >> 20) & 1u) {
            const unsigned grp = (unsigned)wave_read_lane((int)jgrp, (int)s);
            if (lane == 0) {
              const unsigned g0 = S.goff[grp], gn = S.gcnt[grp];
              S.gids[g0 + gn] = (uint16_t)id;
              COMPILER_FENCE();
              st_wg(&S.gcnt[grp], (uint16_t)(gn + 1u));
            }
            wave_sync();
          }
          md = wave_uniform_u32(md);
          if (md == CFM_EPOCH) {
            if (lane == 0) S.misc[CFX_EX_LANE] = s, S.misc[CFX_LOGN] = logn, st_wg(&S.ctrl[0], md);
          }
          CF_PROF_T(p3);
          CF_PROF_ADD(2, p3 - p2);
        }
      } else if (is_class_wave) {
        while (md == 0u) {
#if COOK_HAS_ASM_WALK
          if (one_cls != 0xFFFFFFFFu) {
            const cf_u32x8 LV = {c.lv.v0, c.lv.v1, c.lv.v2, c.lv.v3, c.lv.v4, c.lv.v5, c.lv.v6, c.lv.v7};
            const cf_u32x8 JC = {jc, jm, jmeta, lane, 0u, 0u, 0u, 0u};
#define CF_U(x) wave_uniform_u32((unsigned)(x))
            const unsigned long long hcb = (unsigned long long)__double_as_longlong(u_hTc), hmb = (unsigned long long)__double_as_longlong(u_hTm);
            const cf_u32x8 AR = {CF_U(cook_lds_off(S.board)), CF_U(lw), CF_U(base), CF_U((gen & 15u) << 8), CF_U(u_off), CF_U(u_n), CF_U(cook_lds_off(S.cid)), CF_U(one_cls << 16)};
            const cf_u32x8 A2 = {CF_U(hcb), CF_U(hcb >> 32), CF_U(hmb), CF_U(hmb >> 32), CF_U(rep), CF_U(nrep), CF_U(S.cls[one_cls].kind), CF_BOARD};
            for (;;) {
              cf_u32x8 SC = {CF_U(todo), CF_U(todo >> 32), CF_U(cur_ord), CF_U(ph), CF_U(seen), 3u, 0u, 0u};
              asm volatile(CF_ASM_CLASS_STEP
                           : "+{s[36:43]}"(SC)
                           : "{v[64:71]}"(LV), "{v[72:79]}"(JC), "{s[44:51]}"(AR), "{s[52:59]}"(A2)
                           : "v80", "v81", "v82", "v83", "v84", "v85", "v86", "v87", "v88", "v89", "v90", "v91", "v92", "v93", "v94", "v95", "v96", "v97", "v98", "v99", "s60", "s61", "s62",
                             "s63", "s64", "s65", "s66", "s67", "s68", "s69", "s70", "s71", "s72", "s73", "s74", "s75", "s76", "s77", "s78", "s79", "s80", "s81", "s82", "s83", "vcc", "scc",
                             "memory");
              todo = wave_uniform_u64((unsigned long long)SC[1] << 32 | SC[0]), cur_ord = wave_uniform_u32(SC[2]), ph = wave_uniform_u32(SC[3]);
              const unsigned status = wave_uniform_u32(SC[5]);
              if (status == 0u) continue;
              if (status == 2u) {
                SPIN_PAUSE_NEAR();
                continue;
              }
              break;
            }
#undef CF_U
            WAIT_LDS();
          }
#endif
          CF_PROF_T(q0);
          unsigned mode, hw, cnt;
          {
            const unsigned a0 = ld_wg(&S.ctrl[0]), a1 = ld_wg(&S.ctrl[1]), a2 = ld_wg(&S.ctrl[1u + lw]);
            mode = (unsigned)wave_read_lane((int)a0, 0), hw = (unsigned)wave_read_lane((int)a1, 0), cnt = (unsigned)wave_read_lane((int)a2, 0);
          }
          if (mode != 0u) {
            md = mode;
            break;
          }
          COMPILER_FENCE();
          auto answer = [&](unsigned s, unsigned ord, bool again) {
            const unsigned Jc = (unsigned)wave_read_lane((int)jc, (int)s), Jm = (unsigned)wave_read_lane((int)jm, (int)s), meta = (unsigned)wave_read_lane((int)jmeta, (int)s);
            const unsigned kind = meta & 255u;
            if (!(kind < 32u && ((wk >> kind) & 1u))) return;
            CF_PROF_T(q1);
#ifdef CF_DELAY_C
            __builtin_amdgcn_s_sleep(4);
            if ((ord + rep) % 3u == 0u) __builtin_amdgcn_s_sleep(40);
#endif
            CfEnt* e = &S.board[cf_slot(ord) * 8u + lw];
            const unsigned tag = (base + s) << 12 | (gen & 15u) << 8 | (seen & 255u);
            if (again) {
              const unsigned t0 = ld_wg(&e->tag), p0 = e->pos & 0xFFFFu, c0 = e->cid;
              if (((t0 ^ tag) & ~255u) == 0u) {
                bool stands = (c0 & CF_ENT_NONE) != 0u;
                if (!stands) {
                  const CfFree f0 = S.fcm[p0];
                  const uint32_t cd0 = S.cid[p0];
                  stands = wave_read_lane(((f0.c | f0.m) != 0u && !(cd0 & CF_OCC)) ? 1 : 0, 0) != 0;
                }
                if (stands) {
                  st_lane0_b32(&e->tag, tag);
                  return;
                }
              }
            }
            bool done = false;
            if ((meta >> 12) == 0u && one_cls != 0xFFFFFFFFu) {
              const uint32_t lvL = cf_lv_get(c.lv, (meta >> 8) & 15u);
              const unsigned long long mk = cook_ballot(lvL > Jm);
              if (mk == 0ull) {
                st_lane0_b32(&e->tag, 0xFFFFFFFFu);
                st_lane0_b64(&e->pos, 0u, CF_ENT_NONE);
                st_lane0_b32(&e->tag, tag);
                done = true;
              } else {
                const unsigned ch = (unsigned)__ffsll(mk) - 1u;
                const unsigned pos0 = u_off + 64u * ch, n = u_n - 64u * ch;
                const CfFree f = S.fcm[pos0 + lane];
                const uint32_t cid = S.cid[pos0 + lane];
                const unsigned long long bb = cook_ballot((lane < n) & (f.c >= Jc) & (f.m >= Jm) & !(cid & CF_OCC));
                double fa = 1.0 - ((double)(f.c - Jc) * u_hTc + (double)(f.m - Jm) * u_hTm);
                if (bb != 0ull) {
                  const unsigned long long pm = bb & (0ull - bb);
                  const unsigned long long fb = (unsigned long long)__double_as_longlong(fa);
                  st_mask_b32(&e->tag, pm, 0xFFFFFFFFu);
                  st_mask_b128(&e->fc, pm, f.c, f.m, (unsigned)fb, (unsigned)(fb >> 32));
                  st_mask_b64(&e->pos, pm, (pos0 + lane) | ch << 16, (cid & CF_IDMASK) | one_cls << 16 | ((cid & CF_TIE) ? CF_ENT_AMB : 0u));
                  st_mask_b32(&e->tag, pm, tag);
                  done = true;
                  CF_STAT(++st_scans);
                }
              }
            }
            if (!done) {
              const CfJobU J = job_of(s);
              CfAns a;
              cf_class_answer(S, tl, J, lane, c, a, st_scans, st_tight);
              const unsigned long long fb = (unsigned long long)__double_as_longlong(a.fa);
              st_lane0_b32(&e->tag, 0xFFFFFFFFu);
              st_lane0_b128(&e->fc, a.fc, a.fm, (unsigned)fb, (unsigned)(fb >> 32));
              st_lane0_b64(&e->pos, a.pos | a.ch << 16, a.have ? (a.cid | a.cls << 16 | (a.amb ? CF_ENT_AMB : 0u)) : CF_ENT_NONE);
              st_lane0_b32(&e->tag, tag);
            }
            CF_PROF_T(q2);
            CF_PROF_ADD(0, q1 - q0);
            CF_PROF_ADD(1, q2 - q1);
            CF_PROF_ADD(3, 1);
          };
          if (cnt != seen) {
            seen = cnt;
            CF_STAT(++st_rewinds);
            unsigned long long t2 = walkmask & ~cf_below(hw & 255u);
            unsigned o2 = hw >> 8, p2 = o2;
            while (p2 >= nrep) p2 -= nrep;
            for (; t2 != 0ull && o2 < cur_ord; t2 &= t2 - 1ull, ++o2, p2 = p2 + 1u == nrep ? 0u : p2 + 1u)
              if (p2 == rep && wk != 0u) answer((unsigned)__ffsll(t2) - 1u, o2, true);
          }
          if (cur_ord < (hw >> 8)) {
            todo = walkmask & ~cf_below(hw & 255u);
            cur_ord = hw >> 8;
            ph = cur_ord;
            while (ph >= nrep) ph -= nrep;
          }
          while (todo != 0ull && ph != rep) {
            todo &= todo - 1ull, ++cur_ord;
            ph = ph + 1u == nrep ? 0u : ph + 1u;
          }
          if (todo != 0ull && wk != 0u && cur_ord < (hw >> 8) + CF_BOARD) {
            const unsigned s = (unsigned)__ffsll(todo) - 1u;
            const unsigned ord = cur_ord;
            todo &= todo - 1ull, ++cur_ord;
            ph = ph + 1u == nrep ? 0u : ph + 1u;
            answer(s, ord, false);
            continue;
          }
          if (wk != 0u) SPIN_PAUSE_NEAR();
          else SPIN_PAUSE_IDLE();
          CF_PROF_T(q4);
          CF_PROF_ADD(4, q4 - q0);
          CF_PROF_ADD(5, 1);
        }
      } else {
        while (md == 0u) {
          const unsigned mode = cf_poll(&S.ctrl[0]);
          if (mode != 0u) {
            md = mode;
            break;
          }
          SPIN_PAUSE_IDLE();
        }
      }
      EMU_SITE("classfit: collective");
      WAIT_LDS();
      __syncthreads();
      md = wave_uniform_u32(md);
      if (md == CFM_BATCH_END) {
        batch_done = true;
        if (tid == 0) st_wg(&S.ctrl[0], 0u);
        if (is_class_wave) seen = cf_poll(&S.ctrl[1u + lw]);
        break;
      }
      bool epoch = md == CFM_EPOCH;
      const unsigned s = wave_uniform_u32(S.misc[CFX_EX_LANE]);
      if (md == CFM_EXACT) {
        ++st_exact;
        const double fmax = __longlong_as_double((long long)((unsigned long long)S.misc[CFX_FMAX_LO] | (unsigned long long)S.misc[CFX_FMAX_HI] << 32));
        CfPost mine;
        if (is_decider) {
          const CfJobU J = job_of(s);
          cf_overlay_query_exact(S, J, lane, o, fmax, cf_pow2(-(int)wave_uniform_u32(S.envw[CFE_KC])), cf_pow2(-(int)wave_uniform_u32(S.envw[CFE_KM])), mine);
          if (lane == 0) S.post2[0] = mine;
        } else if (is_class_wave && rep == 0u && lw != 0u) {
          const CfJobU J = job_of(s);
          cf_class_query_exact(S, J, lane, c, fmax, cf_pow2(-(int)wave_uniform_u32(S.envw[CFE_KC])), cf_pow2(-(int)wave_uniform_u32(S.envw[CFE_KM])), mine, st_scans);
          if (lane == 0) S.post2[lw] = mine;
        }
        EMU_SITE("classfit: exact turn");
        __syncthreads();
        if (is_decider) {
          const CfJobU J = job_of(s);
          unsigned used_sets = 0;
          for (unsigned ci = 0; ci < n_cls; ++ci) used_sets |= 1u << wave_uniform_u32(S.cls[ci].wave);
          const CfVerdict v = cf_verdict_exact(S.post2, lane, used_sets);
          const unsigned nfc = v.fc - J.c, nfm = v.fm - J.m;
          const bool dead = nfc < cmin || nfm < mmin;
          const bool from_ov = v.src == 0;
          const bool gpu_place = !from_ov && J.kind != 0u;
          const bool opens = !from_ov && !gpu_place && !dead;
          ++matched;
          if (lane == s) res = (int)v.id;
          b1m |= __ballot((jc > nfc) | (jm > nfm)) & ~cf_below(s) & ~(1ull << s);
          minfc_all = cf_min(minfc_all, nfc), minfm_all = cf_min(minfm_all, nfm);
          unsigned live = (unsigned)__popcll(__ballot(isov && o.valid != 0u));
          unsigned lpos = 0, linfo = s;
          if (from_ov) {
            CF_STAT(++st_ovwin);
            if (lane == v.pos) {
              o.fc = nfc, o.fm = nfm;
              if (dead) o.valid = 0u;
            }
            if (dead) --live;
          } else {
            lpos = v.pos, linfo = s | (unsigned)v.src << 8 | v.aux << 12 | (gpu_place ? 1u : 0u) << 20;
            if (lane == CF_OVL - 1u + (unsigned)v.src) {
              if (gpu_place) S.fcm[lpos] = CfFree{nfc, nfm}, S.cid[lpos] = (uint16_t)(S.cid[lpos] | CF_OCC);
              else S.fcm[lpos] = CfFree{0u, 0u};
              ++nrm, rm2 = rm1, rm1 = lpos;
              S.ctrl[1u + (unsigned)v.src] = nrm;
            }
            if (opens) {
              CF_STAT(++st_open);
              const unsigned lf = (unsigned)__ffsll(~__ballot((isov && o.valid != 0u) || !isov)) - 1u;
              const CfClass* cl = &S.cls[v.cls];
              const double hTc2 = cl->hTc, hTm2 = cl->hTm;
              if (lane == lf) o.valid = 1u, o.id = v.id, o.cls = v.cls, o.fc = nfc, o.fm = nfm, o.hTc = hTc2, o.hTm = hTm2;
              ++live;
            } else if (gpu_place) {
              CF_STAT(++st_gpu);
            } else {
              CF_STAT(++st_opendead);
            }
          }
          if (lane == 0) {
            CfLog* lg = &S.log[logn];
            lg->info = linfo, lg->pos = lpos, lg->ofc = v.fc, lg->ofm = v.fm, lg->nfc = nfc, lg->nfm = nfm;
          }
          ++logn;
          if (J.grouped && lane == 0) {
            const unsigned g0 = S.goff[J.grp], gn = S.gcnt[J.grp];
            S.gids[g0 + gn] = (uint16_t)v.id, S.gcnt[J.grp] = (uint16_t)(gn + 1u);
          }
          todo &= ~(1ull << s), ++cur_ord;
          epoch = opens && live >= CF_EPOCH_AT;
          if (lane == 0) S.misc[CFX_EPOCH] = epoch ? 1u : 0u, S.misc[CFX_LOGN] = logn;
        }
        EMU_SITE("classfit: exact turn done");
        __syncthreads();
        epoch = wave_uniform_u32(S.misc[CFX_EPOCH]) != 0u;
      }
      if (epoch) {
        const unsigned long long te = CF_TICKS();
        ++st_epochs;
        if (is_decider) {
          const bool live = isov && o.valid != 0u;
          const CfClass* cl = &S.cls[live ? o.cls : 0u];
          const unsigned long long key = live ? ((unsigned long long)o.cls << 58 | ((unsigned long long)o.fc * cl->Tm + (unsigned long long)o.fm * cl->Tc) << 13 | (unsigned long long)o.id) : ~0ull;
          unsigned rank = 0;
          for (unsigned l = 0; l < 64u; ++l) rank += wave_read_lane_u64(key, (int)l) < key ? 1u : 0u;
          if (live) S.ovl[3u * rank] = o.cls << 16 | o.id, S.ovl[3u * rank + 1u] = o.fc, S.ovl[3u * rank + 2u] = o.fm;
          const unsigned nlive = (unsigned)__popcll(__ballot(live));
          if (lane == 0) S.misc[CFX_OVN] = nlive;
          if (isov) o.valid = 0u;
          rm1 = rm2 = 0xFFFFFFFFu;
        }
        for (unsigned x = tid; x < 3u * CF_MAXCLS; x += CF_THREADS) S.ckept[x] = 0u;
        EMU_SITE("classfit: epoch 1");
        __syncthreads();
        if (is_class_wave && rep == 0u) {
          unsigned mykept = 0;
          for (unsigned ch = 0; ch < nch_wave; ++ch) {
            const unsigned pos0 = (unsigned)wave_read_lane((int)c.pos0, (int)ch), n = (unsigned)wave_read_lane((int)c.n, (int)ch);
            const CfFree f = S.fcm[pos0 + lane];
            const unsigned kept = (unsigned)__popcll(__ballot(lane < n && (f.c | f.m) != 0u));
            if (lane == ch) mykept = kept;
          }
          if (c.cls != 0xFFu) atomicAdd(&S.ckept[c.cls], mykept);
        }
        if (is_decider && lane < S.misc[CFX_OVN]) atomicAdd(&S.ckept[CF_MAXCLS + (S.ovl[3u * lane] >> 16)], 1u);
        __syncthreads();
        if (tid == 0) {
          unsigned off = 0;
          for (unsigned ci = 0; ci < n_cls; ++ci) S.ckept[2 * CF_MAXCLS + ci] = off, off += S.ckept[ci] + S.ckept[CF_MAXCLS + ci];
        }
        __syncthreads();
        if (is_class_wave && rep == 0u) {
          unsigned li = 0;
          for (unsigned ci = 0; ci < n_cls; ++ci) {
            const unsigned ni = wave_uniform_u32(S.ckept[CF_MAXCLS + ci]);
            if (S.cls[ci].wave == lw) {
              const unsigned noff = wave_uniform_u32(S.ckept[2 * CF_MAXCLS + ci]);
              const unsigned Tc = S.cls[ci].Tc, Tm = S.cls[ci].Tm;
              unsigned kept_before = 0, ip = li;
              const unsigned long long chunks = __ballot(c.cls == ci);
              for (unsigned long long mm = chunks; mm; mm &= mm - 1ull) {
                const unsigned ch = (unsigned)__ffsll(mm) - 1u;
                const unsigned pos0 = (unsigned)wave_read_lane((int)c.pos0, (int)ch), n = (unsigned)wave_read_lane((int)c.n, (int)ch);
                const bool in = lane < n;
                const CfFree f = S.fcm[pos0 + lane];
                const uint32_t fc = f.c, fm = f.m, cid = ci << 16 | (uint32_t)S.cid[pos0 + lane];
                const bool keep = in && (fc | fm) != 0u;
                const unsigned long long Ek = (unsigned long long)fc * Tm + (unsigned long long)fm * Tc;
                const unsigned idq = cid & CF_IDMASK;
                const unsigned long long keepm = __ballot(keep);
                if (keepm == 0ull) continue;
                const unsigned lastk = 63u - (unsigned)__clzll(keepm);
                const unsigned long long Elast = wave_read_lane_u64(Ek, (int)lastk);
                const unsigned idlast = (unsigned)wave_read_lane((int)idq, (int)lastk);
                unsigned ins_before = ip - li;
                while (ip < li + ni) {
                  const unsigned ecid = S.ovl[3u * ip], efc = S.ovl[3u * ip + 1u], efm = S.ovl[3u * ip + 2u];
                  const unsigned long long Ee = (unsigned long long)efc * Tm + (unsigned long long)efm * Tc;
                  const unsigned ide = ecid & CF_IDMASK;
                  if (!(Ee < Elast || (Ee == Elast && ide < idlast))) break;
                  const bool before = keep && (Ek < Ee || (Ek == Ee && idq < ide));
                  const unsigned long long bm = __ballot(before);
                  if (keep && !before) ++ins_before;
                  const unsigned np = noff + kept_before + (unsigned)__popcll(bm) + (ip - li);
                  if (lane == 0) st_agent(&b.scr_fc[np], efc), st_agent(&b.scr_fm[np], efm), st_agent(&b.scr_cid[np], ecid);
                  ++ip;
                }
                if (keep) {
                  const unsigned np = noff + kept_before + (unsigned)__popcll(keepm & lanemask_lt()) + ins_before;
                  st_agent(&b.scr_fc[np], fc), st_agent(&b.scr_fm[np], fm), st_agent(&b.scr_cid[np], cid);
                }
                kept_before += (unsigned)__popcll(keepm);
              }
              for (; ip < li + ni; ++ip) {
                const unsigned np = noff + kept_before + (ip - li);
                if (lane == 0) st_agent(&b.scr_fc[np], S.ovl[3u * ip + 1u]), st_agent(&b.scr_fm[np], S.ovl[3u * ip + 2u]), st_agent(&b.scr_cid[np], S.ovl[3u * ip]);
              }
            }
            li += ni;
          }
        }
        drain_stores();
        EMU_SITE("classfit: epoch 3");
        __syncthreads();
        unsigned newM = 0;
        for (unsigned ci = 0; ci < n_cls; ++ci) newM += S.ckept[ci] + S.ckept[CF_MAXCLS + ci];
        for (unsigned q = tid; q < NP; q += CF_THREADS) {
          const bool inq = q < newM;
          const uint32_t fcq = inq ? ld_agent(&b.scr_fc[q]) : 0u, fmq = inq ? ld_agent(&b.scr_fm[q]) : 0u, cq = inq ? ld_agent(&b.scr_cid[q]) : 0u;
          bool tie = false;
          if (q + 1u < newM) {
            const uint32_t fcn = ld_agent(&b.scr_fc[q + 1u]), fmn = ld_agent(&b.scr_fm[q + 1u]), cn = ld_agent(&b.scr_cid[q + 1u]);
            if ((cn >> 16) == (cq >> 16)) {
              const CfClass* cl = &S.cls[cq >> 16];
              tie = (unsigned long long)fcn * cl->Tm + (unsigned long long)fmn * cl->Tc <= (unsigned long long)fcq * cl->Tm + (unsigned long long)fmq * cl->Tc + cl->dE;
            }
          }
          S.fcm[q] = CfFree{fcq, fmq}, S.cid[q] = inq ? (uint16_t)((cq & (CF_OCC | CF_IDMASK)) | (tie ? CF_TIE : 0u)) : (uint16_t)0u;
        }
        if (tid < n_cls) S.cls[tid].n = S.ckept[tid] + S.ckept[CF_MAXCLS + tid], S.cls[tid].off = S.ckept[2 * CF_MAXCLS + tid];
        EMU_SITE("classfit: epoch 4");
        __syncthreads();
        if (is_class_wave) {
          cf_setup_chunks(S.cls, n_cls, lw, lane, c, nch_wave);
          class_setup();
          for (unsigned ch = 0; ch < nch_wave; ++ch) cf_tighten(S, tl, lane, ch, c);
          if (rep == 0u && lw != 0u) cf_wave_tables(S, lw, lane, c, wk, n_kind);
          tight_applied = st_tight;
        }
        if (tid == 0) S.misc[CFX_LOG_APPLIED] = S.misc[CFX_LOGN];
        tk_epoch += CF_TICKS() - te;
      }
      {
        ++gen;
        if (is_class_wave) {
          todo = walkmask & ~cf_below(s) & ~(1ull << s), cur_ord = (unsigned)__popcll(walkmask & cf_below(s)) + 1u;
          ph = cur_ord;
          while (ph >= nrep) ph -= nrep;
        }
      }
      if (tid == 0) st_wg(&S.ctrl[0], 0u);
      EMU_SITE("classfit: collective done");
      __syncthreads();
      if (is_class_wave) seen = cf_poll(&S.ctrl[1u + lw]);
    }
    tk_walk += CF_TICKS() - tw0;
    CF_PROF_T(cw1);
    CF_PROF_ADD(7, cw1 - cw0);
    const unsigned long long tp0 = CF_TICKS();
    if (is_decider && nw == 0u) decider_books(0u);
    if (nw != 0u) {
      if (is_class_wave) {
        const CfLog* lp = &S.log[lane];
        const unsigned info = lp->info, ofc = lp->ofc, ofm = lp->ofm;
        const unsigned n_log = wave_uniform_u32(S.misc[CFX_LOGN]), a0 = wave_uniform_u32(S.misc[CFX_LOG_APPLIED]);
        const bool mine = lane >= a0 && lane < n_log && ((info >> 8) & 15u) == lw;
        const unsigned ch = (info >> 12) & 63u;
        const unsigned nl = cf_level_of(tl, ofc);
#define CF_LV_AT(i) const unsigned g##i = (unsigned)__shfl((int)c.lv.v##i, (int)ch, COOK_WAVE);
        CF_FOR8(CF_LV_AT)
#undef CF_LV_AT
        bool was_max = ((info >> 20) & 1u) != 0u;
#define CF_WAS_MAX(i) was_max = was_max | (((unsigned)i < nl) & (g##i == ofm + 1u));
        CF_FOR8(CF_WAS_MAX)
#undef CF_WAS_MAX
        unsigned long long stale = 0ull;
        for (unsigned long long fm = cook_ballot(mine & was_max); fm != 0ull; fm &= fm - 1ull) stale |= 1ull << (unsigned)wave_read_lane((int)ch, __ffsll(fm) - 1);
        bool dirty = st_tight != tight_applied;
        for (; stale != 0ull; stale &= stale - 1ull) {
          cf_tighten(S, tl, lane, (unsigned)__ffsll(stale) - 1u, c);
          ++st_tight;
          dirty = true;
        }
        if (dirty && rep == 0u && lw != 0u) cf_wave_tables(S, lw, lane, c, wk, n_kind);
        tight_applied = st_tight;
      }
    }
    EMU_SITE("classfit: phase 2");
    __syncthreads();
    tk_phase1 += CF_TICKS() - tp0;
    if (is_books) {
      const unsigned long long tb0 = CF_TICKS();
      const unsigned long long mm = (unsigned long long)S.misc[CFX_MATCH_LO] | (unsigned long long)S.misc[CFX_MATCH_HI] << 32,
                               bb = (unsigned long long)S.misc[CFX_B1_LO] | (unsigned long long)S.misc[CFX_B1_HI] << 32;
      const unsigned n_log = wave_uniform_u32(S.misc[CFX_LOGN]);
      const CfJob j = S.ring[slot * 64u + (lane < bn ? lane : 0u)];
      const bool unm = lane < bn && !((mm >> lane) & 1ull);
      const unsigned L = (j.meta >> 8) & 15u;
      bool room = unm && tables_room_any(L, j.m);
      const bool flip = unm && !room && bk_room0 && n_log != 0u;
      if (__ballot(flip) != 0ull) {
        ++st_flips;
        for (unsigned x = 0; x < n_log; ++x) {
          const CfLog lg = S.log[x];
          if (flip && (lg.info & 255u) > lane && lg.ofc >= j.c && lg.ofm >= j.m) room = true;
        }
      }
      if (lane < bn && st.fail_code) {
        unsigned fail = 0u;
        if (unm) {
          fail = (((bb >> lane) & 1ull) ? 1u : 0u) | (room ? 2u : 0u);
          if (fail == 0u) fail = 8u;
        }
        st.fail_code[base + lane] = fail;
      }
      unsigned nb = base + 64u;
      unsigned long long nwm = books_next(nb);
      const unsigned minfc_pub = wave_uniform_u32(S.misc[CFX_MINFC]), minfm_pub = wave_uniform_u32(S.misc[CFX_MINFM]);
      while (nb < K && nwm == 0ull) {
        if (nb + lane < K) {
          st.job_to_offer[nb + lane] = -1;
          if (st.fail_code) {
            const unsigned fail = ((nxt.c > minfc_pub || nxt.m > minfm_pub) ? 1u : 0u) | (nx_room0 ? 2u : 0u);
            st.fail_code[nb + lane] = fail != 0u ? fail : 8u;
          }
        }
        books_advance(nb);
        nb += 64u;
        nwm = books_next(nb);
      }
      if (lane == 0) S.misc[CFX_NEXT_BASE] = nb;
      bk_room0 = nx_room0;
      books_advance(nb);
      tk_books += CF_TICKS() - tb0;
    }
    EMU_SITE("classfit: batch end");
    __syncthreads();
    const unsigned nbase = wave_uniform_u32(S.misc[CFX_NEXT_BASE]);
#ifdef CF_PROF
    if (is_class_wave) prof[6] += 16ull * ((nbase - base) / 64u - 1u);
#endif
    base = nbase;
  }
  if (is_decider) {
    if (lane == 0) {
      st.summary[0] = matched;
      st.summary[1] = (matched == 0u || head) ? 1u : 0u;
      st.summary[2] = st_epochs;
      const unsigned long long t_end = cook_ticks();
      uint32_t* sx = ctl->stats;
      sx[CFS_MATCHED] = matched, sx[CFS_OV_WIN] = st_ovwin, sx[CFS_OPEN] = st_open, sx[CFS_OPEN_DEAD] = st_opendead, sx[CFS_GPU_PLACE] = st_gpu, sx[CFS_EPOCHS] = st_epochs,
      sx[CFS_EXACT] = st_exact, sx[CFS_WALKED] = st_walked, sx[CFS_DEAD_DROP] = st_dead, sx[CFS_BATCHES] = (K + 63u) / 64u, sx[CFS_PRESETTLED] = K - st_walked;
      sx[CFS_TICKS_TOTAL] = (uint32_t)(t_end - t_start), sx[CFS_TICKS_PROLOGUE] = (uint32_t)(t_loop - t_start), sx[CFS_TICKS_EPOCH] = (uint32_t)tk_epoch;
      sx[CFS_TICKS_WALK] = (uint32_t)tk_walk, sx[CFS_TICKS_PHASE1] = (uint32_t)tk_phase1;
      sx[CFS_HWID_DECIDER] = cook_hw_id();
    }
    const unsigned sp = wave_max_u32(!isov ? st_spins : 0u);
    if (lane == 0) ctl->stats[CFS_SPINS] = sp;
  }
  if (is_class_wave && lane == 0) atomicAdd(&ctl->stats[CFS_SCANS], st_scans), atomicAdd(&ctl->stats[CFS_TIGHTEN], st_tight), atomicAdd(&ctl->stats[CFS_REWINDS], st_rewinds);
  if (is_books && lane == 0) ctl->stats[CFS_TICKS_PRECHECK] = (uint32_t)tk_books, ctl->stats[CFS_FLIPS] = st_flips, ctl->stats[CFS_HWID_BOOKS] = cook_hw_id();
#ifdef CF_PROF
  if (lane == 0 && (is_decider || (is_class_wave && lw >= 1u && lw <= 2u && rep == 0u)))
    for (int i = 0; i < 8; ++i) ctl->stats[24 + 8 * (is_decider ? 0u : lw) + i] = (uint32_t)(prof[i] >> 4);
#endif
#undef n_cls
#undef n_kind
#undef NP
}

static __device__ __forceinline__ void cf_walk_pool(char* lds, const MatchIn* __restrict__ inp, const MatchState& st, const CfBuf& b) {
  const unsigned tid = threadIdx.x, lane = lane_id(), w = wave_id();
  CfCtl* ctl = b.ctl;
  const unsigned K = inp->K, M = ctl->M, G = inp->G;
  const unsigned NP = (M + 63u) & ~63u;
  const unsigned long long t_start = cook_ticks();
  const bool any_eq = ctl->any_eq != 0u, any_group = ctl->any_group != 0u;
  __shared__ unsigned s_total, s_wsum[CF_WAVES];
  static_assert(CF_MAXG % CF_THREADS == 0, "the groups are dealt out GPT to a thread: a workgroup size that does not divide CF_MAXG would leave some without one");
  constexpr unsigned GPT = CF_MAXG / CF_THREADS;
  unsigned gsz[GPT];
  unsigned gsum = 0;
#pragma unroll
  for (unsigned x = 0; x < GPT; ++x) {
    const unsigned g = tid * GPT + x;
    unsigned sz = 0;
    if (any_group && g < G && b.gcount[g] != 0u) sz = (inp->g_run_off ? inp->g_run_off[g + 1] - inp->g_run_off[g] : 0u) + b.gcount[g];
    gsz[x] = sz, gsum += sz;
  }
  unsigned incl = gsum;
  for (unsigned d = 1; d < 64u; d <<= 1) {
    const unsigned y = shfl_up_t<unsigned>(incl, d);
    if (lane >= d) incl += y;
  }
  if (lane == 63u) s_wsum[w] = incl;
  __syncthreads();
  unsigned wbase = 0;
  for (unsigned x = 0; x < w; ++x) wbase += s_wsum[x];
  if (tid == CF_THREADS - 1) s_total = wbase + incl;
  __syncthreads();
  const unsigned Stot = any_group ? s_total : 0u, Gl = any_group ? G : 0u;
  CfLds S;
  {
    CfFixed* F = (CfFixed*)lds;
    S.board = F->board, S.log = F->log, S.ring = F->ring, S.post2 = F->post2, S.cls = F->cls, S.pw = F->pw, S.aw = F->aw, S.gk = F->gk, S.ovt = F->ovt, S.ctrl = F->ctrl, S.ovl = F->ovl,
    S.ckept = F->ckept, S.misc = F->misc, S.t = F->env_t, S.envw = F->envw;
    char* p = lds + sizeof(CfFixed);
    S.fcm = (CfFree*)p, p += NP * 8u;
    S.cid = (uint16_t*)p, p += NP * 2u;
    p = lds + (((unsigned)(p - lds) + 7u) & ~7u);
    S.attr8 = (uint64_t*)p;
    if (any_eq) p += M * 8u;
    S.goff = (uint16_t*)p, p += (Gl + 1u) * 2u;
    S.gcnt = (uint16_t*)p, p += Gl * 2u;
    S.gids = (uint16_t*)p, p += Stot * 2u;
    if ((unsigned)(p - lds) > CF_LDS_BYTES) {
      if (tid == 0) atomicOr(&ctl->inelig, (unsigned)CF_X_SHAPE), st.summary[3] = 0xDEADu;
      return;
    }
  }
#ifdef CF_DIAG_CLEAR_LDS
  for (unsigned x = tid; x < CF_LDS_BYTES / 4u; x += CF_THREADS) ((uint32_t*)lds)[x] = 0u;
  __syncthreads();
#endif
  for (unsigned q = tid; q < NP; q += CF_THREADS) {
    S.fcm[q] = q < M ? CfFree{b.pos_fc[q], b.pos_fm[q]} : CfFree{0u, 0u}, S.cid[q] = q < M ? (uint16_t)b.pos_cid[q] : (uint16_t)0u;
  }
  if (any_eq)
    for (unsigned v = tid; v < M; v += CF_THREADS) S.attr8[v] = b.attr8[v];
  if (any_group) {
    unsigned off = wbase + incl - gsum;
#pragma unroll
    for (unsigned x = 0; x < GPT; ++x) {
      const unsigned g = tid * GPT + x;
      if (g <= G) S.goff[g] = (uint16_t)off;
      if (g < G) {
        unsigned cnt = 0;
        if (gsz[x]) {
          const unsigned r0 = inp->g_run_off ? inp->g_run_off[g] : 0u, r1 = inp->g_run_off ? inp->g_run_off[g + 1] : 0u;
          for (unsigned r = r0; r < r1; ++r) {
            const uint32_t h = inp->g_run_host[r];
            const uint32_t v = h <= b.max_host ? b.h2o[h] : 0xFFFFFFFFu;
            if (v != 0xFFFFFFFFu) S.gids[off + cnt++] = (uint16_t)v;
          }
        }
        S.gcnt[g] = (uint16_t)cnt;
        off += gsz[x];
      }
    }
  }
  {
    CfFixed* F = (CfFixed*)lds;
    if (tid < (unsigned)CF_LV) F->env_t[tid] = ctl->t[tid];
    if (tid == 0) {
      uint32_t* ew = F->envw;
      ew[CFE_K] = K, ew[CFE_M] = M, ew[CFE_NP] = NP, ew[CFE_NCLS] = ctl->n_cls, ew[CFE_NKIND] = ctl->n_kind, ew[CFE_CMIN] = ctl->cmin, ew[CFE_MMIN] = ctl->mmin, ew[CFE_KC] = ctl->kc,
      ew[CFE_KM] = ctl->km, ew[CFE_MINFC] = ctl->minfc_all, ew[CFE_MINFM] = ctl->minfm_all;
    }
  }
  for (unsigned x = tid; x < ctl->n_cls; x += CF_THREADS) S.cls[x] = ctl->cls[x];
  for (unsigned x = tid; x < CFX_N; x += CF_THREADS) S.misc[x] = 0u;
  for (unsigned x = tid; x < 8u * CF_LV; x += CF_THREADS) S.pw[x] = 0u, S.aw[x] = 0u;
  for (unsigned x = tid; x < 8u; x += CF_THREADS) S.ctrl[x] = 0u;
  for (unsigned x = tid; x < CF_MAXKIND * CF_LV; x += CF_THREADS) S.gk[x] = 0u;
  for (unsigned x = tid; x < (unsigned)CF_LV; x += CF_THREADS) S.ovt[x] = 0u;
  for (unsigned x = tid; x < CF_SLOTS * 8u; x += CF_THREADS) S.board[x].tag = 0xFFFFFFFFu;
  __syncthreads();
  if (w == 0u) {
    cf_walk_role<0>(S, st, b, 0u, 0u, 1u, t_start);
  } else if (w == CFW_BOOKS) {
    cf_walk_role<2>(S, st, b, 0u, 0u, 1u, t_start);
  } else {
    const unsigned p = w < CFW_BOOKS ? w - 1u : w - 2u, np = (unsigned)CF_WAVES - 2u;
    unsigned used = 0, zsets = 0;
    for (unsigned ci = 0; ci < ctl->n_cls; ++ci) {
      const unsigned g = S.cls[ci].wave;
      used |= 1u << g;
      if (S.cls[ci].kind == 0u) zsets |= 1u << g;
    }
    used = wave_uniform_u32(used), zsets = wave_uniform_u32(zsets);
    unsigned myset = 0, rep = 0, nrep = 0, k = 0;
    for (unsigned pass = 0; pass < np && k < np; ++pass) {
      const unsigned from = pass == 0u ? used : (zsets ? zsets : used);
      if (from == 0u) break;
      for (unsigned g = 1; g <= (unsigned)CF_CW && k < np; ++g)
        if ((from >> g) & 1u) {
          if (k == p) myset = g;
          ++k;
        }
    }
    k = 0;
    for (unsigned pass = 0; pass < np && k < np; ++pass) {
      const unsigned from = pass == 0u ? used : (zsets ? zsets : used);
      if (from == 0u) break;
      for (unsigned g = 1; g <= (unsigned)CF_CW && k < np; ++g)
        if ((from >> g) & 1u) {
          if (g == myset) {
            if (k < p) ++rep;
            ++nrep;
          }
          ++k;
        }
    }
    if (nrep == 0u) nrep = 1u;
    {
      const unsigned cap = nrep >= 12u ? 12u : nrep >= 6u ? 6u : nrep == 5u ? 4u : nrep;
      if (rep >= cap) myset = 0u, rep = 0u, nrep = 1u;
      else nrep = cap;
    }
    cf_walk_role<1>(S, st, b, wave_uniform_u32(myset), wave_uniform_u32(rep), wave_uniform_u32(nrep), t_start);
  }
}
```

Before: 22.40.

## Run decider todo loop entirely inside inline asm instead of per-step C++ loop

The decider wave's loop over pending slots moves from a C++ while-loop that called one asm step per slot into a single asm block that loops internally. It uses s_ff1 on the todo mask, advances the board offset, order and log pointer in scalar registers, and exits only on status change. The cross-lane max reduction is interleaved with scalar bookkeeping so the DPP hazard nops are filled with useful work, and a few redundant address computations are folded. This is meant to cut per-slot re-entry overhead (argument repacking, readfirstlane, register moves), at the cost of harder-to-verify state handoff between the asm and C++ code. Profiling counters are also extended.

```diff
diff --git a/cook_amd/csrc/classfit_asm.hpp b/cook_amd/csrc/classfit_asm.hpp
--- a/cook_amd/csrc/classfit_asm.hpp
+++ b/cook_amd/csrc/classfit_asm.hpp
@@ -6,6 +6,7 @@
 #define CF_O_CLS32 "9504"
 #define CF_SLOT_SHIFT "9"
 #define CF_SLOT_N "12"
+#define CF_ROW_END "3072"
 #elif CF_SLOTS_N == 24
 #define CF_O_CTRL "16800"
 #define CF_O_CTRL4 "16804"
@@ -13,27 +14,41 @@
 #define CF_O_CLS32 "12576"
 #define CF_SLOT_SHIFT "10"
 #define CF_SLOT_N "24"
+#define CF_ROW_END "6144"
 #else
 #error "CF_SLOTS_N: 12 or 24"
 #endif
 #ifndef CF_ASM_WAIT_READS
 #define CF_ASM_WAIT_READS "30"
 #endif
-#define CF_ASM_MAX_STEP(ctrl) "v_max_f32_dpp v113, v113, v113 " ctrl "\n\ts_nop 1\n\t"
-#define CF_ASM_DECIDER_STEP                                                                                                             \
-  "v_readlane_b32 s60, v80, s44\n\t"                                                                                                    \
-  "v_readlane_b32 s61, v81, s44\n\t"                                                                                                    \
-  "v_readlane_b32 s62, v82, s44\n\t"                                                                                                    \
-  "s_mov_b32 s41, 1\n\t"                                                                                                                \
-  "s_and_b32 s63, s62, 0xffff00ff\n\t"                                                                                                   \
-  "s_cmp_lg_u32 s63, 0\n\t"                                                                                                             \
-  "s_cbranch_scc1 9f\n\t"                                                                                                               \
+#ifdef CF_DELAY_D
+#define CF_ASM_DELAY_D "s_sleep 6\n\t"
+#else
+#define CF_ASM_DELAY_D
+#endif
+#define CF_ASM_DECIDER_RUN \
+   \
+  "v_lshl_add_u32 v114, v65, 3, s56\n\t" \
+  "ds_read_b64 v[114:115], v114\n\t" \
+  "s_ff1_i32_b64 s44, s[42:43]\n\t" \
+  "s_lshl_b32 s45, s44, 12\n\t" \
+  "s_add_u32 s45, s45, s59\n\t" \
+  "s_lshl_b32 s47, s57, 8\n\t" \
+  "s_or_b32 s47, s47, s44\n\t" \
+  "s_mov_b32 s41, 1\n\t"  \
+   \
+  "0:\n\t" \
+  "v_readlane_b32 s60, v80, s44\n\t" \
+  "v_readlane_b32 s61, v81, s44\n\t" \
+  "v_readlane_b32 s62, v82, s44\n\t" \
+  "s_and_b32 s63, s62, 0xffff00ff\n\t"  \
+  "s_cmp_lg_u32 s63, 0\n\t" \
+  "s_cbranch_scc1 9f\n\t" \
                                                                                            \
   "v_mov_b32_e32 v88, s47\n\t"                                                                                                          \
-  "v_mov_b32_e32 v89, s51\n\t"                                                                                                          \
   "v_add_u32_e32 v100, s46, v83\n\t"                                                                                                    \
   "s_mov_b64 exec, 1\n\t"                                                                                                               \
-  "ds_write_b32 v89, v88 offset:" CF_O_CTRL4 "\n\t"                                                                                              \
+  "ds_write_b32 v87, v88 offset:" CF_O_CTRL4 "\n\t"                                                                                              \
   "s_mov_b64 exec, -1\n\t"                                                                                                              \
   "s_mov_b32 s82, " CF_ASM_WAIT_READS "\n\t"              \
   "1:\n\t"                                                                                                                              \
@@ -41,9 +56,6 @@
   "ds_read_b64 v[94:95], v100 offset:8\n\t"                                                                                             \
   "ds_read_b128 v[96:99], v100 offset:16\n\t"                                                                                           \
   "ds_read_b32 v93, v100\n\t"                                                                                                           \
-  "v_lshlrev_b32_e32 v114, 3, v65\n\t"  \
-  "v_add_u32_e32 v114, s56, v114\n\t"                                                                                                   \
-  "ds_read_b64 v[114:115], v114\n\t"                                                                                                    \
                                         \
   "v_subrev_u32_e32 v101, s60, v71\n\t"                                                                                                 \
   "v_subrev_u32_e32 v102, s61, v72\n\t"                                                                                                 \
@@ -160,26 +172,37 @@
   "v_cndmask_b32_e64 v111, v99, v105, s[54:55]\n\t"                                                                                     \
   "v_cndmask_b32_e64 v110, 0, v110, s[64:65]\n\t"                                                                                       \
   "v_cndmask_b32_e64 v111, 0, v111, s[64:65]\n\t"                                                                                       \
-  "v_cvt_f32_f64_e32 v112, v[110:111]\n\t"                                                                                              \
-  "s_nop 0\n\t"                                                                                                                         \
-  "v_mov_b32_e32 v113, v112\n\t"                                                                                                        \
-  "s_nop 1\n\t"                                                                                                                         \
-  CF_ASM_MAX_STEP("quad_perm:[1,0,3,2] row_mask:0xf bank_mask:0xf")                                                                     \
-  CF_ASM_MAX_STEP("quad_perm:[2,3,0,1] row_mask:0xf bank_mask:0xf")                                                                     \
-  CF_ASM_MAX_STEP("row_half_mirror row_mask:0xf bank_mask:0xf")                                                                         \
-  CF_ASM_MAX_STEP("row_mirror row_mask:0xf bank_mask:0xf")                                                                              \
-  CF_ASM_MAX_STEP("row_bcast:15 row_mask:0xa bank_mask:0xf")                                                                            \
-  CF_ASM_MAX_STEP("row_bcast:31 row_mask:0xc bank_mask:0xf")                                                                            \
-  "v_readlane_b32 s63, v113, 63\n\t"                                                                                                    \
-  "s_mov_b32 s41, 0\n\t"                                                                                                                \
-  "s_cmp_eq_u32 s63, 0\n\t"                                                                                                             \
-  "s_cbranch_scc1 9f\n\t"                                                                                          \
-  "s_mov_b32 s41, 1\n\t"                                                                                                                \
-  "v_cmp_eq_f32_e64 s[78:79], s63, v112\n\t"                                                                                            \
-  "v_add_f32_e32 v108, 0x35000000, v112\n\t"                                                                               \
-  "v_cmp_le_f32_e64 s[76:77], s63, v108\n\t"                                                                                            \
-  "v_and_b32_e32 v109, 0x40000000, v95\n\t"                                                                                             \
-  "v_cmp_ne_u32_e64 s[70:71], 0, v109\n\t"                                                                                              \
+  "v_cvt_f32_f64_e32 v112, v[110:111]\n\t" \
+   \
+   \
+   \
+  "s_mov_b64 s[84:85], s[42:43]\n\t" \
+  "v_mov_b32_e32 v113, v112\n\t" \
+  "s_bitset0_b64 s[84:85], s44\n\t" \
+  "s_add_u32 s46, s46, 256\n\t" \
+  "v_max_f32_dpp v113, v113, v113 quad_perm:[1,0,3,2] row_mask:0xf bank_mask:0xf\n\t" \
+  "s_ff1_i32_b64 s86, s[84:85]\n\t" \
+  "s_add_u32 s62, s57, 1\n\t" \
+  "v_max_f32_dpp v113, v113, v113 quad_perm:[2,3,0,1] row_mask:0xf bank_mask:0xf\n\t" \
+  "s_cmp_eq_u32 s46, " CF_ROW_END "\n\t" \
+  "s_cselect_b32 s46, 0, s46\n\t" \
+  "v_max_f32_dpp v113, v113, v113 row_half_mirror row_mask:0xf bank_mask:0xf\n\t" \
+  "s_lshl_b32 s62, s62, 8\n\t" \
+  "s_or_b32 s47, s62, s86\n\t" \
+  "v_max_f32_dpp v113, v113, v113 row_mirror row_mask:0xf bank_mask:0xf\n\t" \
+  "s_lshl_b32 s63, s86, 12\n\t" \
+  "s_add_u32 s45, s59, s63\n\t" \
+  "v_max_f32_dpp v113, v113, v113 row_bcast:15 row_mask:0xa bank_mask:0xf\n\t" \
+  "v_add_f32_e32 v108, 0x35000000, v112\n\t" \
+  "v_and_b32_e32 v109, 0x40000000, v95\n\t" \
+  "v_max_f32_dpp v113, v113, v113 row_bcast:31 row_mask:0xc bank_mask:0xf\n\t" \
+  "v_cmp_ne_u32_e64 s[70:71], 0, v109\n\t" \
+  "s_nop 0\n\t" \
+  "v_readlane_b32 s63, v113, 63\n\t" \
+  "s_cmp_eq_u32 s63, 0\n\t" \
+  "s_cbranch_scc1 8f\n\t"  \
+  "v_cmp_eq_f32_e64 s[78:79], s63, v112\n\t" \
+  "v_cmp_le_f32_e64 s[76:77], s63, v108\n\t"  \
   "s_and_b64 s[76:77], s[76:77], s[64:65]\n\t"                                      \
   "s_bcnt1_i32_b64 s62, s[76:77]\n\t"                                                                                                   \
   "s_cmp_gt_u32 s62, 1\n\t"                                                                                                             \
@@ -200,11 +223,10 @@
   "v_cmp_eq_u32_e64 vcc, s82, v84\n\t"                                                                                                  \
   "v_mov_b32_e32 v88, s67\n\t"                                                                                                          \
   "v_mov_b32_e32 v89, s70\n\t"                                                                                                          \
-  "s_cmp_lt_u32 s67, s49\n\t"                                                                                                           \
-  "s_cselect_b32 s71, 1, 0\n\t"                                                                                                         \
-  "s_cmp_lt_u32 s70, s50\n\t"                                                                                                           \
-  "s_cselect_b32 s62, 1, 0\n\t"                                                                                                         \
-  "s_or_b32 s71, s71, s62\n\t"                                                                                                          \
+  "s_cmp_lt_u32 s67, s49\n\t" \
+  "s_cselect_b32 s71, 1, 0\n\t" \
+  "s_cmp_lt_u32 s70, s50\n\t" \
+  "s_cselect_b32 s71, 1, s71\n\t" \
   "v_cndmask_b32_e32 v71, v71, v88, vcc\n\t"                                                                                            \
   "v_cndmask_b32_e32 v72, v72, v89, vcc\n\t"                                                                                            \
   "s_cmp_lg_u32 s71, 0\n\t"                                                                                                             \
@@ -227,51 +249,48 @@
   "s_and_b32 s73, s77, 0xffff\n\t"                                                                                                      \
   "s_lshr_b32 s81, s77, 16\n\t"                                                                                                         \
   "s_sub_u32 s80, s82, 57\n\t"                                                                                                          \
-  "s_cmp_lt_u32 s67, s49\n\t"                                                                                                           \
-  "s_cselect_b32 s71, 1, 0\n\t"                                                                                                         \
-  "s_cmp_lt_u32 s70, s50\n\t"                                                                                                           \
-  "s_cselect_b32 s62, 1, 0\n\t"                                                                                                         \
-  "s_or_b32 s71, s71, s62\n\t"                                                                                                          \
+  "s_cmp_lt_u32 s67, s49\n\t" \
+  "s_cselect_b32 s71, 1, 0\n\t" \
+  "s_cmp_lt_u32 s70, s50\n\t" \
+  "s_cselect_b32 s71, 1, s71\n\t" \
   "s_bcnt1_i32_b64 s62, s[68:69]\n\t"                                                                                                   \
   "s_cmp_lg_u32 s71, 0\n\t"                                                                                                             \
   "s_cbranch_scc1 6f\n\t"                                                                                                               \
   "s_cmp_ge_u32 s62, " CF_ASM_EPOCH_LIVE "\n\t"                                                                                          \
   "s_cbranch_scc1 9f\n\t"                                  \
   "6:\n\t"                                                                                                                              \
-  "s_lshl_b32 s62, s73, 3\n\t"                                                                                                          \
-  "s_add_u32 s62, s62, s51\n\t"                                                                                                         \
-  "s_lshl_b32 s63, s80, 2\n\t"                                                                                                          \
-  "s_add_u32 s63, s63, s51\n\t"                                                                                                         \
-  "s_add_u32 s78, s78, 1\n\t"                                                                                                           \
-  "v_mov_b32_e32 v88, 0\n\t"                                                                                                            \
-  "v_mov_b32_e32 v89, 0\n\t"                                                                                                            \
-  "v_mov_b32_e32 v90, s62\n\t"                                                                                                          \
-  "v_mov_b32_e32 v91, s63\n\t"                                                                                                          \
+  "s_lshl_b32 s62, s73, 3\n\t" \
+  "s_lshl_b32 s63, s80, 2\n\t" \
+  "s_add_u32 s78, s78, 1\n\t" \
+  "v_mov_b32_e32 v88, 0\n\t" \
+  "v_mov_b32_e32 v89, 0\n\t" \
+  "v_add_u32_e32 v90, s62, v87\n\t" \
+  "v_add_u32_e32 v91, s63, v87\n\t" \
   "v_mov_b32_e32 v100, s78\n\t"                                                                                                         \
   "s_mov_b64 exec, 1\n\t"                                                                                                               \
   "ds_write_b64 v90, v[88:89] offset:" CF_O_ARR "\n\t"                                                                                         \
   "ds_write_b32 v91, v100 offset:" CF_O_CTRL4 "\n\t"                                                                                             \
   "s_mov_b64 exec, -1\n\t"                                                                                                              \
   "v_cmp_eq_u32_e64 vcc, s82, v84\n\t"                                                                                                  \
-  "v_mov_b32_e32 v101, s73\n\t"                                                                                                         \
-  "s_nop 0\n\t"                                                                                                                         \
-  "v_cndmask_b32_e32 v75, v75, v74, vcc\n\t"                                                                                            \
-  "v_cndmask_b32_e32 v74, v74, v101, vcc\n\t"                                                                                           \
-  "v_cndmask_b32_e32 v73, v73, v100, vcc\n\t"                                                                                           \
-  "s_lshl_b32 s62, s80, 8\n\t"                                                                                                          \
+  "v_mov_b32_e32 v101, s73\n\t" \
+  "s_lshl_b32 s62, s80, 8\n\t" \
+  "v_cndmask_b32_e32 v75, v75, v74, vcc\n\t" \
+  "v_cndmask_b32_e32 v74, v74, v101, vcc\n\t" \
+  "v_cndmask_b32_e32 v73, v73, v100, vcc\n\t" \
   "s_lshl_b32 s63, s81, 12\n\t"                                                                                                         \
   "s_or_b32 s72, s44, s62\n\t"                                                                                                          \
   "s_or_b32 s72, s72, s63\n\t"                                                                                                          \
   "s_cmp_lg_u32 s71, 0\n\t"                                                                                                             \
   "s_cbranch_scc1 7f\n\t"                                                                              \
-  "s_mul_i32 s62, s79, 56\n\t"                                                                                                          \
-  "s_add_u32 s62, s62, s51\n\t"                                                                                                         \
-  "v_mov_b32_e32 v90, s62\n\t"                                                                                                          \
-  "ds_read_b128 v[116:119], v90 offset:" CF_O_CLS32 "\n\t"                                                                                        \
+  "s_mul_i32 s62, s79, 56\n\t" \
+  "v_add_u32_e32 v90, s62, v87\n\t" \
+  "ds_read_b128 v[116:119], v90 offset:" CF_O_CLS32 "\n\t"  \
+  "v_mov_b32_e32 v88, s66\n\t" \
+  "v_lshl_add_u32 v102, v88, 3, s56\n\t"   \
+  "ds_read_b64 v[102:103], v102\n\t"                                                                                        \
   "s_andn2_b64 s[62:63], s[54:55], s[68:69]\n\t"                                                                                        \
   "s_ff1_i32_b64 s83, s[62:63]\n\t"                                                                                                     \
   "v_cmp_eq_u32_e64 vcc, s83, v84\n\t"                                                                                                  \
-  "v_mov_b32_e32 v88, s66\n\t"                                                                                                          \
   "v_mov_b32_e32 v89, s79\n\t"                                                                                                          \
   "v_mov_b32_e32 v91, s67\n\t"                                                                                                          \
   "v_mov_b32_e32 v101, s70\n\t"                                                                                                         \
@@ -284,7 +303,9 @@
   "v_cndmask_b32_e32 v66, v66, v116, vcc\n\t"                                                                                           \
   "v_cndmask_b32_e32 v67, v67, v117, vcc\n\t"                                                                                           \
   "v_cndmask_b32_e32 v68, v68, v118, vcc\n\t"                                                                                           \
-  "v_cndmask_b32_e32 v69, v69, v119, vcc\n\t"                                                                                           \
+  "v_cndmask_b32_e32 v69, v69, v119, vcc\n\t"  \
+  "v_cndmask_b32_e32 v114, v114, v102, vcc\n\t" \
+  "v_cndmask_b32_e32 v115, v115, v103, vcc\n\t"                                                                                           \
    \
   "7:\n\t"                                                                                                                              \
   "v_cmp_eq_u32_e64 vcc, s44, v84\n\t"                                                                                                  \
@@ -302,13 +323,22 @@
   "v_mov_b32_e32 v88, s72\n\t"                                                                                                          \
   "v_mov_b32_e32 v89, s73\n\t"                                                                                                          \
   "v_mov_b32_e32 v90, s64\n\t"                                                                                                          \
-  "v_mov_b32_e32 v91, s65\n\t"                                                                                                          \
-  "v_mov_b32_e32 v100, s48\n\t"                                                                                                         \
-  "s_mov_b64 exec, 1\n\t"                                                                                                               \
-  "ds_write_b128 v100, v[88:91]\n\t"                                                                                                    \
-  "s_mov_b64 exec, -1\n\t"                                                                                                              \
-  "s_mov_b32 s41, 2\n\t"                                                                                                                \
-  "9:\n\t"
+  "v_mov_b32_e32 v91, s65\n\t" \
+  "s_mov_b64 exec, 1\n\t" \
+  "ds_write_b128 v77, v[88:91]\n\t" \
+  "s_mov_b64 exec, -1\n\t" \
+  "v_add_u32_e32 v77, 32, v77\n\t"  \
+   \
+  "8:\n\t" \
+  CF_ASM_DELAY_D \
+  "s_mov_b64 s[42:43], s[84:85]\n\t" \
+  "s_mov_b32 s44, s86\n\t" \
+  "s_add_u32 s57, s57, 1\n\t" \
+  "s_cmp_lg_u64 s[42:43], 0\n\t" \
+  "s_cbranch_scc1 0b\n\t" \
+  "s_mov_b32 s41, 0\n\t" \
+  "9:\n\t" \
+  "s_waitcnt lgkmcnt(0)\n\t"
 
 #define CF_ASM_CLASS_STEP                                                                                                               \
   "v_mov_b32_e32 v80, s44\n\t"                                                                                                          \
diff --git a/cook_amd/csrc/classfit_host.hpp b/cook_amd/csrc/classfit_host.hpp
--- a/cook_amd/csrc/classfit_host.hpp
+++ b/cook_amd/csrc/classfit_host.hpp
@@ -61,6 +61,7 @@
 static void cf_prof_print(const uint32_t* q) {
 #ifdef CF_PROF
   std::fprintf(stderr, "CFPROF (x16 shader cycles) decider: slow steps %u (candidates %u evaluation %u commit %u) plain steps %u in %u walk-total %u | class wave 1: poll %u answer %u answers %u idle %u idles %u | class wave 2: poll %u answer %u answers %u idle %u idles %u | walk ticks(100MHz) %u | batch boundaries: decider %u, batches without a walked job %u\n", q[27], q[24], q[25], q[26], q[28], q[29], q[31], q[32], q[33], q[35], q[36], q[37], q[40], q[41], q[43], q[44], q[45], q[CFS_TICKS_WALK], q[30], q[38]);
+  std::fprintf(stderr, "CFPROF plain steps %u, C++ steps %u; steps that left the plain form: gpu kind %u, novel hosts %u, group %u, answer missing after the re-reads %u, guard band %u, epoch end %u\n", q[46], q[47], q[34] & 65535u, q[34] >> 16, q[39] & 65535u, q[39] >> 16, q[42] & 65535u, q[42] >> 16);
 #else
   (void)q;
 #endif
diff --git a/cook_amd/csrc/classfit_walk.hpp b/cook_amd/csrc/classfit_walk.hpp
--- a/cook_amd/csrc/classfit_walk.hpp
+++ b/cook_amd/csrc/classfit_walk.hpp
@@ -12,9 +12,13 @@
 #ifdef CF_PROF
 #define CF_PROF_T(x) const unsigned long long x = __builtin_readcyclecounter()
 #define CF_PROF_ADD(i, d) prof[i] += (unsigned long long)(d)
+#define CF_PROF_WHY(n) why = why == 3u ? (n) : why
+#define CF_PROF_LEAVE() (why < 4u ? leave_a += 1ull << (16u * why) : leave_b += 1ull << (16u * (why - 4u)))
 #else
 #define CF_PROF_T(x) ((void)0)
 #define CF_PROF_ADD(i, d) ((void)0)
+#define CF_PROF_WHY(n) ((void)0)
+#define CF_PROF_LEAVE() ((void)0)
 #endif
 
 #ifndef CF_AHEAD
@@ -342,6 +346,7 @@
 #define CF_ASM_EPOCH_LIVE "57"
 #include "classfit_asm.hpp"
 static_assert(CF_EPOCH_AT == 58 && CF_OVL == 58, "classfit_asm.hpp: the overlay's size");
+static_assert(sizeof(CfEnt) * 8u == 256u && sizeof(CfEnt) * 8u * CF_SLOTS == 3072u + (CF_SLOTS - 12u) * 256u, "classfit_asm.hpp: a row of the board is 256 bytes, CF_ROW_END the board's size");
 static_assert(offsetof(CfFixed, ctrl) == 13728 + (CF_SLOTS - 12) * 256 && offsetof(CfFixed, cls) == 9472 + (CF_SLOTS - 12) * 256 && sizeof(CfFixed) == 15280 + (CF_SLOTS - 12) * 256 && sizeof(CfClass) == 56 && offsetof(CfClass, hTc) == 32 &&
                   offsetof(CfClass, hTm) == 40 && offsetof(CfEnt, pos) == 8 && offsetof(CfEnt, cid) == 12 && offsetof(CfEnt, fc) == 16 && offsetof(CfEnt, fa) == 24 && sizeof(CfEnt) == 32 &&
                   sizeof(CfLog) == 32 && offsetof(CfLog, ofc) == 8,
@@ -406,6 +411,7 @@
   unsigned long long tk_epoch = 0, tk_books = 0, tk_walk = 0, tk_phase1 = 0;
 #ifdef CF_PROF
   unsigned long long prof[8] = {0, 0, 0, 0, 0, 0, 0, 0}, bnd0 = 0ull;
+  unsigned long long leave_a = 0ull, leave_b = 0ull;
 #endif
   auto job_of = [&](unsigned s) -> CfJobU {
     CfJobU J;
@@ -523,15 +529,13 @@
       if (is_decider) {
 #if COOK_HAS_ASM_WALK
         cf_u32x16 ST = {0u, 0u, 0u, 0u, 0u, 0u, 0u, 0u, 0u, 0u, 0u, 0u, 0u, 0u, 0u, 0u};
-        cf_u32x8 JB = {jc, jm, jmeta, clw * 32u, lane, jeq0, jeq1, 0u};
+        const unsigned a_board = wave_uniform_u32(cook_lds_off(S.board)), a_log = wave_uniform_u32(cook_lds_off(S.log));
+        cf_u32x8 JB = {jc, jm, jmeta, a_board + clw * (unsigned)sizeof(CfEnt), lane, jeq0, jeq1, a_board};
         const unsigned long long rel0 = cook_ballot(!isov & ((my_kinds & 1u) != 0u)), ovm = cf_below(CF_OVL);
-        const cf_u32x8 MK = {wave_uniform_u32((unsigned)rel0), wave_uniform_u32((unsigned)(rel0 >> 32)), wave_uniform_u32((unsigned)ovm), wave_uniform_u32((unsigned)(ovm >> 32)),
-                             wave_uniform_u32(cook_lds_off(S.attr8)), 0u, 0u, 0u};
-        const unsigned a_board = wave_uniform_u32(cook_lds_off(S.board)), a_log = wave_uniform_u32(cook_lds_off(S.log));
         auto st_pack = [&] {
           const unsigned long long hc = (unsigned long long)__double_as_longlong(o.hTc), hm = (unsigned long long)__double_as_longlong(o.hTm);
           ST[0] = o.valid, ST[1] = o.id, ST[2] = (unsigned)hc, ST[3] = (unsigned)(hc >> 32), ST[4] = (unsigned)hm, ST[5] = (unsigned)(hm >> 32), ST[6] = o.cls, ST[7] = o.fc, ST[8] = o.fm,
-          ST[9] = nrm, ST[10] = rm1, ST[11] = rm2, ST[12] = (unsigned)res;
+          ST[9] = nrm, ST[10] = rm1, ST[11] = rm2, ST[12] = (unsigned)res, ST[13] = a_log + logn * (unsigned)sizeof(CfLog);
         };
         auto st_unpack = [&] {
           o.valid = ST[0], o.id = ST[1], o.hTc = __longlong_as_double((long long)((unsigned long long)ST[3] << 32 | ST[2])),
@@ -543,33 +547,26 @@
           todo = wave_uniform_u64(todo), cur_ord = wave_uniform_u32(cur_ord), logn = wave_uniform_u32(logn), matched = wave_uniform_u32(matched), gen = wave_uniform_u32(gen);
           minfc_all = wave_uniform_u32(minfc_all), minfm_all = wave_uniform_u32(minfm_all), b1m = wave_uniform_u64(b1m);
 #if COOK_HAS_ASM_WALK
-          {
+          if (todo != 0ull) {
             st_pack();
             CF_PROF_T(f0);
-            while (todo != 0ull) {
-              const unsigned fs = (unsigned)__ffsll(todo) - 1u;
 #define CF_U(x) wave_uniform_u32((unsigned)(x))
-              cf_u32x8 SC = {CF_U(matched), CF_U(minfc_all), CF_U(b1m), CF_U(b1m >> 32), CF_U(minfm_all), 1u, 0u, 0u};
-              const cf_u32x8 AR = {CF_U(fs), CF_U((base + fs) << 12 | (gen & 15u) << 8), CF_U(a_board + cf_slot(cur_ord) * 8u * (unsigned)sizeof(CfEnt)), CF_U(fs | cur_ord << 8),
-                                   CF_U(a_log + logn * (unsigned)sizeof(CfLog)), CF_U(cmin), CF_U(mmin), a_board};
+            cf_u32x8 SC = {CF_U(matched), CF_U(minfc_all), CF_U(b1m), CF_U(b1m >> 32), CF_U(minfm_all), 1u, CF_U(todo), CF_U(todo >> 32)};
+            cf_u32x8 AR = {0u, 0u, CF_U(cf_slot(cur_ord) * 8u * (unsigned)sizeof(CfEnt)), 0u, 0u, CF_U(cmin), CF_U(mmin), a_board};
+            cf_u32x8 MK = {CF_U(rel0), CF_U(rel0 >> 32), CF_U(ovm), CF_U(ovm >> 32), CF_U(cook_lds_off(S.attr8)), CF_U(cur_ord), 0u, CF_U(base << 12 | (gen & 15u) << 8)};
+            asm volatile(CF_ASM_DECIDER_RUN
+                         : "+{v[64:79]}"(ST), "+{s[36:43]}"(SC), "+{s[44:51]}"(AR), "+{s[52:59]}"(MK)
+                         : "{v[80:87]}"(JB)
+                         : "v88", "v89", "v90", "v91", "v92", "v93", "v94", "v95", "v96", "v97", "v98", "v99", "v100", "v101", "v102", "v103", "v104", "v105", "v106", "v107", "v108",
+                           "v109", "v110", "v111", "v112", "v113", "v114", "v115", "v116", "v117", "v118", "v119", "s60", "s61", "s62", "s63", "s64", "s65", "s66", "s67", "s68", "s69",
+                           "s70", "s71", "s72", "s73", "s74", "s75", "s76", "s77", "s78", "s79", "s80", "s81", "s82", "s83", "s84", "s85", "s86", "vcc", "scc", "memory");
+            matched = CF_U(SC[0]), minfc_all = CF_U(SC[1]), minfm_all = CF_U(SC[4]);
+            b1m = wave_uniform_u64((unsigned long long)SC[3] << 32 | SC[2]);
+            todo = wave_uniform_u64((unsigned long long)SC[7] << 32 | SC[6]);
+            logn = (CF_U(ST[13]) - a_log) / (unsigned)sizeof(CfLog);
+            CF_PROF_ADD(4, CF_U(MK[5]) - cur_ord);
+            cur_ord = CF_U(MK[5]);
 #undef CF_U
-              asm volatile(CF_ASM_DECIDER_STEP
-                           : "+{v[64:79]}"(ST), "+{s[36:43]}"(SC)
-                           : "{v[80:87]}"(JB), "{s[44:51]}"(AR), "{s[52:59]}"(MK)
-                           : "v88", "v89", "v90", "v91", "v92", "v93", "v94", "v95", "v96", "v97", "v98", "v99", "v100", "v101", "v102", "v103", "v104", "v105", "v106", "v107", "v108",
-                             "v109", "v110", "v111", "v112", "v113", "v114", "v115", "v116", "v117", "v118", "v119", "s60", "s61", "s62", "s63", "s64", "s65", "s66", "s67", "s68", "s69",
-                             "s70", "s71", "s72", "s73", "s74", "s75", "s76", "s77", "s78", "s79", "s80", "s81", "s82", "s83", "vcc", "scc", "memory");
-#ifdef CF_DELAY_D
-              __builtin_amdgcn_s_sleep(6);
-#endif
-              const unsigned status = wave_uniform_u32(SC[5]);
-              if (status == 1u) break;
-              matched = wave_uniform_u32(SC[0]), minfc_all = wave_uniform_u32(SC[1]), minfm_all = wave_uniform_u32(SC[4]);
-              b1m = wave_uniform_u64((unsigned long long)SC[3] << 32 | SC[2]);
-              logn += status >> 1;
-              todo &= todo - 1ull, ++cur_ord;
-              CF_PROF_ADD(4, 1);
-            }
             CF_PROF_T(f1);
             CF_PROF_ADD(5, f1 - f0);
             WAIT_LDS();
@@ -592,6 +589,9 @@
           const unsigned Jc = (unsigned)wave_read_lane((int)jc, (int)s), Jm = (unsigned)wave_read_lane((int)jm, (int)s), meta = (unsigned)wave_read_lane((int)jmeta, (int)s);
           const unsigned kind = meta & 255u;
           const unsigned want = (base + s) << 12 | (gen & 15u) << 8;
+#ifdef CF_PROF
+          unsigned why = kind != 0u ? 0u : ((meta >> 16) & 15u) ? 1u : ((meta >> 20) & 1u) ? 2u : 3u;
+#endif
           const CfEnt* e = &S.board[cf_slot(ord) * 8u + clw];
           const bool relevant = !isov && kind < 32u && ((my_kinds >> (kind & 31u)) & 1u);
           unsigned cpos, ccid, cfc, cfm;
@@ -638,11 +638,13 @@
           CF_PROF_ADD(1, p2 - p1);
           CF_PROF_ADD(3, 1);
           if (!(mx > 0.0f)) {
+            CF_PROF_LEAVE();
             todo &= todo - 1ull, ++cur_ord;
             continue;
           }
           unsigned l0 = (unsigned)__ffsll(eqm) - 1u;
           if ((nearm & (nearm - 1ull)) != 0ull || ambm != 0ull) {
+            CF_PROF_WHY(4u);
             const unsigned long long mxb = wave_max_u64((unsigned long long)__double_as_longlong(fa));
             const double f0 = __longlong_as_double((long long)mxb);
             l0 = (unsigned)__ffsll(__ballot(ok && (unsigned long long)__double_as_longlong(fa) == mxb)) - 1u;
@@ -651,6 +653,7 @@
             if (amb) {
               md = CFM_EXACT;
               if (lane == 0) S.misc[CFX_EX_LANE] = s, S.misc[CFX_FMAX_LO] = (unsigned)mxb, S.misc[CFX_FMAX_HI] = (unsigned)(mxb >> 32), st_wg(&S.ctrl[0], md);
+              CF_PROF_LEAVE();
               break;
             }
           }
@@ -715,8 +718,10 @@
           }
           md = wave_uniform_u32(md);
           if (md == CFM_EPOCH) {
+            CF_PROF_WHY(5u);
             if (lane == 0) S.misc[CFX_EX_LANE] = s, S.misc[CFX_LOGN] = logn, st_wg(&S.ctrl[0], md);
           }
+          CF_PROF_LEAVE();
           CF_PROF_T(p3);
           CF_PROF_ADD(2, p3 - p2);
         }
@@ -1199,7 +1204,10 @@
   if (is_books && lane == 0) ctl->stats[CFS_TICKS_PRECHECK] = (uint32_t)tk_books, ctl->stats[CFS_FLIPS] = st_flips, ctl->stats[CFS_HWID_BOOKS] = cook_hw_id();
 #ifdef CF_PROF
   if (lane == 0 && (is_decider || (is_class_wave && lw >= 1u && lw <= 2u && rep == 0u)))
-    for (int i = 0; i < 8; ++i) ctl->stats[24 + 8 * (is_decider ? 0u : lw) + i] = (uint32_t)(prof[i] >> 4);
+    for (int i = 0; i < 8; ++i)
+      if (is_decider || (i != 2 && i != 7 && !(lw == 2u && i == 6))) ctl->stats[24 + 8 * (is_decider ? 0u : lw) + i] = (uint32_t)(prof[i] >> 4);
+  if (lane == 0 && is_decider)
+    ctl->stats[34] = (uint32_t)leave_a, ctl->stats[39] = (uint32_t)(leave_a >> 32), ctl->stats[42] = (uint32_t)leave_b, ctl->stats[46] = (uint32_t)prof[4], ctl->stats[47] = (uint32_t)prof[3];
 #endif
 #undef n_cls
 #undef n_kind
```

Measured after the change: 23.34, median of 6. +4.2%, better.
